# SciML/ExponentialUtilities.jl

Hardware: AMD Instinct MI355X
Metric: expv matvecs/s (Krylov steps/s), n=1e6 5-diagonal sparse fp64, m=30 (higher is better)
Workload: dtype f64; 1 GPU; BASELINE configs[1]: expv(1.0, A, b), n=1000000, offsets (-2..2) diagonals (0.3,1.2,-2.0,0.8,-0.1), nnz=4999994, m=30, tol=1e-7, full Arnoldi (auto), one independent problem per GPU; n=1000000, m=30, nnz=4999994, ortho=auto, entry=expv(t,A,b), outputs=stream-ordered, spinup_calls=535

## Files before the change

### exponentialutilities.jl_amd/_lib.py

```python
import ctypes as C
import os

HERE = os.path.dirname(os.path.abspath(__file__))
LIB_PATH = os.environ.get("EXPV_MI_LIB") or os.path.join(HERE, "libexpv_mi.so")

F64, C64, F32, C32 = 0, 1, 2, 3
HOST, DEVICE = 0, 1
ORTHO_AUTO, ORTHO_MGS, ORTHO_LOWSYNC, ORTHO_PIPELINED = 0, 1, 2, 3
PATH_FLAGS = {"modular": 1, "two_kernel": 2, "pipeline": 4, "wave": 8, "overlapped": 16, "redo_serial": 32,
              "redo_wave_off": 64, "resident": 128, "patch": 256, "pipelined_lanczos": 512}
PATH_FA2_PIPELINED = 1024

STATUS_NAMES = {
    0: "OK", 1: "DimensionMismatch", 2: "ArgumentError", 3: "AssertionError", 4: "SingularException",
    5: "Unsupported", 6: "OutOfMemory", 7: "HIPError", 8: "BoundsError",
}

KERNEL_IDS = {"firststep": 0, "matvec": 1, "dots": 2, "update": 3, "scale": 4, "combine": 5,
              "fused_a": 6, "fused_b": 7, "lincomb": 8, "aug": 9, "batch": 10}


class ArnoldiOpts(C.Structure):
    _fields_ = [("m", C.c_int32), ("iop", C.c_int32), ("init", C.c_int32), ("ishermitian", C.c_int32),
                ("ortho", C.c_int32), ("flags", C.c_int32), ("tol", C.c_double)]


class ExpvStats(C.Structure):
    _fields_ = [("m_used", C.c_int32), ("wasbreakdown", C.c_int32), ("matvecs", C.c_int32),
                ("path_flags", C.c_int32), ("beta", C.c_double)]


ABI_KINDS = {"ArnoldiOpts": 0, "ExpvStats": 1, "TimestepOpts": 2, "TimestepStats": 3, "KiopsOpts": 4}
PRINT_FN = C.CFUNCTYPE(None, C.c_char_p, C.c_void_p)
MATVEC_FN = C.CFUNCTYPE(C.c_int, C.c_void_p, C.c_void_p, C.c_void_p, C.c_void_p)


class TimestepOpts(C.Structure):
    _fields_ = [("tau", C.c_double), ("tol", C.c_double), ("delta", C.c_double), ("gamma", C.c_double),
                ("opnorm", C.c_double), ("has_opnorm", C.c_int32), ("m", C.c_int32), ("iop", C.c_int32),
                ("correct", C.c_int32), ("adaptive", C.c_int32), ("ishermitian", C.c_int32),
                ("verbose", C.c_int32), ("ortho", C.c_int32), ("no_basis_reuse", C.c_int32), ("reserved", C.c_int32),
                ("NA", C.c_int64), ("print", PRINT_FN),
                ("print_user", C.c_void_p)]


class TimestepStats(C.Structure):
    _fields_ = [("num_timesteps", C.c_int32), ("matvecs", C.c_int32), ("m_final", C.c_int32),
                ("arnoldi_calls", C.c_int32), ("arnoldi_reused", C.c_int32), ("stalled_steps", C.c_int32)]


class KiopsOpts(C.Structure):
    _fields_ = [("mmin", C.c_int32), ("mmax", C.c_int32), ("m", C.c_int32), ("iop", C.c_int32),
                ("ishermitian", C.c_int32), ("task1", C.c_int32), ("ortho", C.c_int32),
                ("reserved", C.c_int32), ("tol", C.c_double)]


_vp, _i, _i64, _d = C.c_void_p, C.c_int, C.c_int64, C.c_double
_pi, _pi64, _pd, _pvp = C.POINTER(C.c_int), C.POINTER(C.c_int64), C.POINTER(C.c_double), C.POINTER(C.c_void_p)
PROTOTYPES = {
    "expv_mi_ctx_create": (_i, [_i, _vp, _pvp]),
    "expv_mi_ctx_destroy": (_i, [_vp]),
    "expv_mi_ctx_sync": (_i, [_vp]),
    "expv_mi_ctx_set_async_outputs": (_i, [_vp, _i]),
    "expv_mi_ctx_set_pipeline_overlap": (_i, [_vp, _i]),
    "expv_mi_ctx_counters": (_i, [_vp, _pi64]),
    "expv_mi_ctx_selftest": (_i, [_vp, _pi64]),
    "expv_mi_ctx_set_option": (_i, [_vp, C.c_char_p, _i64]),
    "expv_mi_ctx_get_option": (_i, [_vp, C.c_char_p, _pi64]),
    "expv_mi_last_error": (C.c_char_p, [_vp]),
    "expv_mi_version": (C.c_char_p, []),
    "expv_mi_malloc": (_i, [_vp, C.c_size_t, _pvp]),
    "expv_mi_free": (_i, [_vp, _vp]),
    "expv_mi_memcpy_h2d": (_i, [_vp, _vp, _vp, C.c_size_t]),
    "expv_mi_memcpy_d2h": (_i, [_vp, _vp, _vp, C.c_size_t]),
    "expv_mi_prof_enable": (_i, [_vp, _i]),
    "expv_mi_prof_reset": (_i, [_vp]),
    "expv_mi_prof_get": (_i, [_vp, _i, _pi64, _pd]),
    "expv_mi_prof_name": (C.c_char_p, [_i]),
    "expv_mi_op_create_csc": (_i, [_vp, _i, _i64, _vp, _vp, _vp, _i, _pvp]),
    "expv_mi_op_create_csr": (_i, [_vp, _i, _i64, _vp, _vp, _vp, _i, _i, _pvp]),
    "expv_mi_op_create_csr_loc": (_i, [_vp, _i, _i64, _i64, _vp, _vp, _vp, _i, _i, _i, _pvp]),
    "expv_mi_op_create_csc_loc": (_i, [_vp, _i, _i64, _i64, _vp, _vp, _vp, _i, _i, _i, _pvp]),
    "expv_mi_op_create_coo_loc": (_i, [_vp, _i, _i64, _i64, _vp, _vp, _vp, _i, _i, _i, _pvp]),
    "expv_mi_op_ingest_info": (_i, [_vp, _vp]),
    "expv_mi_op_create_dense": (_i, [_vp, _i, _i64, _vp, _i64, _i, _pvp]),
    "expv_mi_op_create_callback": (_i, [_vp, _i, _i64, MATVEC_FN, _vp, _i, _i64, _pvp]),
    "expv_mi_op_destroy": (_i, [_vp]),
    "expv_mi_op_update_values": (_i, [_vp, _vp, _i]),
    "expv_mi_op_info": (_i, [_vp, _pi64, _pi64, _pi, _pd, _pi]),
    "expv_mi_op_reorder_info": (_i, [_vp, _vp]),
    "expv_mi_op_patch_info": (_i, [_vp, _vp]),
    "expv_mi_plan_cache": (_i, [_i, _i64, _vp]),
    "expv_mi_host_patch_order": (_i, [C.c_int64, _vp, _vp, _i, _vp, _vp, _vp]),
    "expv_mi_host_mesh_patch_order": (_i, [C.c_int64, _vp, _vp, _i, _vp, _vp, _vp]),
    "expv_mi_op_apply": (_i, [_vp, _vp, _i, _vp, _i]),
    "expv_mi_gemv_block": (_i, [_vp, _i, _i64, _i64, _vp, _i64, _vp, _vp, _vp, _i]),
    "expv_mi_expm": (_i, [_vp, _i, _i64, _vp, _i64, _i, _vp]),
    "expv_mi_expm_balanced": (_i, [_vp, _i, _i64, _vp, _i64, _i, _vp]),
    "expv_mi_gebal": (_i, [_vp, _i, _i64, _vp, _i64, _i, _vp, _vp, _vp]),
    "expv_mi_phi": (_i, [_vp, _i, _i64, _i, _vp, _i64, _vp, _i64, _i, _vp]),
    "expv_mi_gemm": (_i, [_vp, _i, _i64, _i64, _i64, _d, _d, _vp, _i64, _vp, _i64, _d, _d, _vp, _i64]),
    "expv_mi_ks_create": (_i, [_vp, _i, _i, _i64, _i, _i, _pvp]),
    "expv_mi_ks_destroy": (_i, [_vp]),
    "expv_mi_ks_resize": (_i, [_vp, _i]),
    "expv_mi_ks_get": (_i, [_vp, _pi, _pi, _pi, _pd, _pi]),
    "expv_mi_ks_set_m": (_i, [_vp, _i]),
    "expv_mi_ks_H": (_i, [_vp, _pvp, _pi, _pi, _pi]),
    "expv_mi_ks_V_download": (_i, [_vp, _i, _i, _vp, _i64]),
    "expv_mi_ks_V_upload": (_i, [_vp, _i, _i, _vp, _i64]),
    "expv_mi_ks_V_devptr": (_i, [_vp, _pvp, _pi64]),
    "expv_mi_arnoldi_opts_default": (None, [C.POINTER(ArnoldiOpts)]),
    "expv_mi_arnoldi": (_i, [_vp, _vp, _vp, _i, C.POINTER(ArnoldiOpts)]),
    "expv_mi_lanczos": (_i, [_vp, _vp, _vp, _i, C.POINTER(ArnoldiOpts)]),
    "expv_mi_arnoldi_aug": (_i, [_vp, _vp, _vp, _i64, _i, _i, _vp, _i, _pd, _d, _d, C.POINTER(ArnoldiOpts)]),
    "expv_mi_expv_ks": (_i, [_vp, _d, _d, _vp, _i, _i]),
    "expv_mi_phiv_ks": (_i, [_vp, _d, _d, _i, _i, _vp, _i64, _i, _i, _pd]),
    "expv_mi_combine": (_i, [_vp, _i, _i, _vp, _i, _i, _d, _vp, _i64, _i, _i]),
    "expv_mi_expv": (_i, [_vp, _vp, _d, _d, _vp, _i, _vp, _i, _i, C.POINTER(ArnoldiOpts), C.POINTER(ExpvStats)]),
    "expv_mi_expv_error_estimate": (_i, [_vp, _vp, _d, _d, _vp, _i, _vp, _i, _d, _d, _i, _i]),
    "expv_mi_timestep_opts_default": (None, [C.POINTER(TimestepOpts)]),
    "expv_mi_timestep_caches_create": (_i, [_vp, _i, _i64, _i, _i, _pvp]),
    "expv_mi_timestep_caches_destroy": (_i, [_vp]),
    "expv_mi_phiv_timestep": (_i, [_vp, _vp, _i, _pd, _vp, _i64, _i, _i, _vp, _i64, _i, C.POINTER(TimestepOpts),
                                   _vp, C.POINTER(TimestepStats)]),
    "expv_mi_kiops_opts_default": (None, [C.POINTER(KiopsOpts)]),
    "expv_mi_kiops": (_i, [_vp, _vp, _pd, _i, _i, _vp, _i64, _i, _i, _vp, _i64, _i, C.POINTER(KiopsOpts), _pi64]),
    "expv_mi_expv_batch": (_i, [_vp, _i, _i64, _i, _vp, _vp, _vp, _i64, _i, _pd, _vp, _i64, _i, _vp, _i64, _i,
                                C.POINTER(ArnoldiOpts), C.POINTER(C.c_int32)]),
    "expv_mi_expv_batch_multi": (_i, [_pvp, _i, _i, _i64, _i, _vp, _vp, _vp, _i64, _pd, _vp, _i64, _vp, _i64, _i,
                                      C.POINTER(ArnoldiOpts), C.POINTER(C.c_int32)]),
    "expv_mi_rccl_available": (_i, []),
    "expv_mi_rccl_unique_id": (_i, [_vp]),
    "expv_mi_comm_create": (_i, [_vp, _vp, _i, _i, _pvp]),
    "expv_mi_gather_rccl": (_i, [_vp, _vp, _vp, _i64, _i]),
    "expv_mi_comm_destroy": (_i, [_vp]),
    "expv_mi_abi_sizeof": (C.c_size_t, [_i]),
    "expv_mi_abi_layout": (C.c_char_p, [_i]),
    "expv_mi_host_pattern_info": (_i, [C.c_int64, _vp, _vp, _i, _vp]),
    "expv_mi_host_rcm": (_i, [C.c_int64, _vp, _vp, _i, _vp, _vp]),
    "expv_mi_host_wrapsum": (_i, [_vp, C.c_uint64, _vp]),
    "expv_mi_host_expm": (_i, [_i, _i, _vp, _i]),
    "expv_mi_host_gebal": (_i, [_i, _i, _vp, _i, _vp, _vp, _vp]),
    "expv_mi_host_symtridiag_expcol": (_i, [_i, _pd, _pd, _d, _d, _pd]),
    "expv_mi_host_symtridiag_exp_last": (_i, [_i, _pd, _pd, _d, _d, _pd]),
    "expv_mi_host_phiv_dense": (_i, [_i, _i, _i, _vp, _i, _vp, _vp]),
}

_lib = None


class ExpvMIError(RuntimeError):
    def __init__(self, code, msg):
        super().__init__(f"{STATUS_NAMES.get(code, code)}: {msg}")
        self.code = code
        self.kind = STATUS_NAMES.get(code, str(code))


def load():
    global _lib
    if _lib is not None:
        return _lib
    if not os.path.exists(LIB_PATH):
        raise ImportError(
            f"{LIB_PATH} is missing: build the HIP extension first "
            "(python -c 'import __graft_entry__ as g; g.build()').  There is no CPU fallback.")
    try:
        import torch
    except ImportError:
        pass
    lib = C.CDLL(LIB_PATH)
    for name, (res, args) in PROTOTYPES.items():
        fn = getattr(lib, name)
        fn.restype = res
        fn.argtypes = args
    _lib = lib
    return lib


def check(code, ctx=None):
    if code != 0:
        msg = load().expv_mi_last_error(ctx)
        raise ExpvMIError(code, msg.decode() if msg else "")
```

### exponentialutilities.jl_amd/api.py

```python
import ctypes as C
import math
import os
import weakref

import numpy as np

from . import _lib as L

__all__ = [
    "Context", "default_context", "MIOperator", "DeviceArray", "KrylovSubspace", "arnoldi", "arnoldi_",
    "lanczos_", "expv", "expv_", "phiv", "phiv_", "expv_timestep", "expv_timestep_", "phiv_timestep",
    "phiv_timestep_", "kiops", "timestep_caches", "expv_batch", "expv_batch_multi", "RcclComm", "rccl_available", "rccl_unique_id", "ExpvMIError", "DimensionMismatch", "host_expm",
    "exponential", "exponential_", "mul_", "phi", "phi_", "balance_", "host_gebal",
    "host_phiv_dense", "host_symtridiag_expcol", "host_symtridiag_exp_last", "host_pattern_info", "host_rcm", "host_patch_order", "clear_operator_cache", "plan_cache",
]

ExpvMIError = L.ExpvMIError


class DimensionMismatch(ValueError):
    """Julia's DimensionMismatch (arnoldi.jl:217-218) -- raised for status 1."""


def _check(code, ctx=None):
    if code == 0:
        return
    try:
        L.check(code, ctx)
    except L.ExpvMIError as e:
        if e.code == 1:
            raise DimensionMismatch(str(e)) from None
        if e.code == 3:
            raise AssertionError(str(e)) from None
        if e.code == 8:
            raise IndexError(str(e)) from None
        raise


class Context:


    def __init__(self, device=None, stream=None, async_outputs=False):
        sptr = None
        if stream is not None:
            handle = getattr(stream, "cuda_stream", stream)
            if not handle:
                raise ValueError("Context(stream=...): the null / legacy stream (handle 0, e.g. torch.cuda.default_stream()) cannot be "
                                 "adopted -- the library would silently work on a stream of its own.  Pass a stream you created "
                                 "(torch.cuda.Stream()), or stream=None for a private stream of the library's.")
            sptr = C.c_void_p(int(handle))
        lib = L.load()
        if device is None:
            device = int(os.environ.get("LOCAL_RANK", "0"))
        h = C.c_void_p()
        _check(lib.expv_mi_ctx_create(int(device), sptr, C.byref(h)))
        self._h = h
        self.device = int(device)
        self._stream_keepalive = stream
        self._finalizer = weakref.finalize(self, lib.expv_mi_ctx_destroy, h)
        self._async_outputs = bool(async_outputs)
        if async_outputs:
            _check(lib.expv_mi_ctx_set_async_outputs(h, 1))

    def sync(self):
        _check(L.load().expv_mi_ctx_sync(self._h), self._h)

    def set_async_outputs(self, on=True):
        _check(L.load().expv_mi_ctx_set_async_outputs(self._h, int(bool(on))), self._h)
        self._async_outputs = bool(on)

    def set_option(self, name, value):
        _check(L.load().expv_mi_ctx_set_option(self._h, name.encode(), int(value)), self._h)

    def get_option(self, name):
        v = C.c_int64(0)
        _check(L.load().expv_mi_ctx_get_option(self._h, name.encode(), C.byref(v)), self._h)
        return int(v.value)

    def selftest(self):
        out = (C.c_int64 * 8)()
        _check(L.load().expv_mi_ctx_selftest(self._h, out), self._h)
        return tuple(int(x) for x in out)

    def counters(self):
        out = (C.c_int64 * 8)()
        _check(L.load().expv_mi_ctx_counters(self._h, out), self._h)
        keys = ("krylov_steps", "factorisations", "pipeline", "overlapped", "redo_serial", "redo_wave_off", "op_applies", "h_by_copy")
        return dict(zip(keys, (int(v) for v in out)))

    def set_pipeline_overlap(self, on=True):
        _check(L.load().expv_mi_ctx_set_pipeline_overlap(self._h, int(bool(on))), self._h)

    def prof_enable(self, on=True):
        L.load().expv_mi_prof_enable(self._h, int(bool(on)))

    def prof_reset(self):
        _check(L.load().expv_mi_prof_reset(self._h), self._h)

    def prof_get(self):
        out = {}
        for name, kid in L.KERNEL_IDS.items():
            n, ms = C.c_int64(0), C.c_double(0.0)
            _check(L.load().expv_mi_prof_get(self._h, kid, C.byref(n), C.byref(ms)), self._h)
            if n.value:
                out[name] = {"launches": int(n.value), "total_ms": float(ms.value)}
        return out


_default_ctx = None


def default_context():
    global _default_ctx
    if _default_ctx is None:
        _default_ctx = Context()
    return _default_ctx


class DeviceArray:

    def __init__(self, shape, dtype, ctx=None):
        self.ctx = ctx or default_context()
        self.shape = tuple(int(s) for s in (shape if isinstance(shape, (tuple, list)) else (shape,)))
        self.dtype = np.dtype(dtype)
        nbytes = int(np.prod(self.shape)) * self.dtype.itemsize
        p = C.c_void_p()
        _check(L.load().expv_mi_malloc(self.ctx._h, nbytes, C.byref(p)), self.ctx._h)
        self.ptr = p.value
        self.nbytes = nbytes
        self._finalizer = weakref.finalize(self, L.load().expv_mi_free, self.ctx._h, p)

    @classmethod
    def from_host(cls, a, ctx=None):
        a = np.asfortranarray(a)
        d = cls(a.shape, a.dtype, ctx)
        _check(L.load().expv_mi_memcpy_h2d(d.ctx._h, d.ptr, a.ctypes.data, a.nbytes), d.ctx._h)
        return d

    def to_host(self):
        out = np.empty(self.shape, dtype=self.dtype, order="F")
        _check(L.load().expv_mi_memcpy_d2h(self.ctx._h, out.ctypes.data, self.ptr, self.nbytes), self.ctx._h)
# ... 1357 lines not shown
    if x.dim() != 2 or _dense_np_dtype(x) != dt:
        raise TypeError(f"mul_: {what} must be a 2-D tensor of dtype {dt}")
    return None, None, tuple(x.shape), x


def mul_(Cm, A, B, alpha=1, beta=0, ctx=None):
    dt = _dense_np_dtype(Cm)
    args = [_dense_dev_arg(x, dt, w) for x, w in ((Cm, "C"), (A, "A"), (B, "B"))]
    (m, n), (ma, k), (kb, nb) = (tuple(int(v) for v in a[2]) for a in args)
    if ma != m or kb != k or nb != n:
        raise DimensionMismatch(f"mul!: C is {m}x{n}, A is {ma}x{k}, B is {kb}x{nb}")
    alpha, beta = complex(alpha), complex(beta)
    if dt.kind != "c" and (alpha.imag != 0 or beta.imag != 0):
        raise TypeError("InexactError: complex scalar with a real element type")
    ptrs, keep = [], []
    for i, (ptr, ld, shape, x) in enumerate(args):
        if ptr is None:
            if not (x.stride(0) == 1 and (shape[1] <= 1 or x.stride(1) >= max(shape[0], 1))) and min(shape) > 0:
                if i == 0:
                    raise TypeError("output matrix must be column-major (e.g. torch.empty(n, m).t())")
                x = x.t().contiguous().t()
            keep.append(x)
            ptr, ld = x.data_ptr(), (x.stride(1) if shape[1] > 1 else max(shape[0], 1))
        ptrs.append((ptr, max(int(ld), 1)))
    tens = [x for x in keep if _is_torch(x)]
    if tens:
        _torch_ready(*tens)
    c = ctx or (Cm.ctx if isinstance(Cm, DeviceArray) else default_context())
    _check(L.load().expv_mi_gemm(c._h, _code(dt), m, n, k, alpha.real, alpha.imag, ptrs[1][0], ptrs[1][1], ptrs[2][0], ptrs[2][1],
                                 beta.real, beta.imag, ptrs[0][0], ptrs[0][1]), c._h)
    if not getattr(c, "_async_outputs", False):
        c.sync()
    return Cm


def _host_dtype(*dts):
    dt = np.result_type(*[np.dtype(d) for d in dts])
    if dt.kind not in "fc" or dt.itemsize < 4:
        dt = np.result_type(dt, np.float64)
    if dt.itemsize > 16 or (dt.kind == "f" and dt.itemsize > 8):
        dt = np.dtype(np.complex128 if dt.kind == "c" else np.float64)
    if dt == np.dtype(np.float16):
        dt = np.dtype(np.float32)
    return dt


def host_expm(A):
    A = np.array(A, dtype=_host_dtype(np.asarray(A).dtype), order="F", copy=True)
    n = A.shape[0]
    _check(L.load().expv_mi_host_expm(_HOST_CODES[A.dtype], n, A.ctypes.data, max(n, 1)))
    return A


def host_gebal(A):
    A = np.array(A, dtype=_host_dtype(np.asarray(A).dtype), order="F", copy=True)
    if A.ndim != 2 or A.shape[0] != A.shape[1]:
        raise DimensionMismatch(f"host_gebal: matrix is not square: dimensions are {A.shape}")
    n = A.shape[0]
    ilo, ihi = C.c_int64(1), C.c_int64(0)
    scale = np.ones(n, dtype=np.float64)
    _check(L.load().expv_mi_host_gebal(_HOST_CODES[A.dtype], n, A.ctypes.data, max(n, 1), C.byref(ilo), C.byref(ihi), scale.ctypes.data))
    return A, int(ilo.value), int(ihi.value), scale


def host_pattern_info(A, dtype=np.float64):
    import scipy.sparse as sp
    A = sp.csr_matrix(A)
    n = A.shape[0]
    rp = np.ascontiguousarray(A.indptr, dtype=np.int32)
    ci = np.ascontiguousarray(A.indices, dtype=np.int32)
    out = np.zeros(8, dtype=np.int64)
    _check(L.load().expv_mi_host_pattern_info(n, rp.ctypes.data, ci.ctypes.data, _code(np.dtype(dtype)), out.ctypes.data))
    info = {"sell": bool(out[0]), "bandwidth": int(out[1]), "pipeline_dia_diagonals": int(out[2]),
            "general_dia_diagonals": int(out[3]), "general_dia_max_offset": int(out[4]), "sell_wave_reach": int(out[5]),
            "rows_sorted_unique": bool(out[6]), "sell_cut": int(out[7])}
    if not info["sell"]:
        info["path"] = "modular (empty operator)"
    elif info["sell_cut"] > 0:
        info["path"] = "two-kernel step, SELL slots up to the cut + overflow pass (irregular rows)"
    elif info["pipeline_dia_diagonals"] or (np.dtype(dtype) in (np.dtype(np.float64), np.dtype(np.float32)) and info["bandwidth"] <= 8):
        info["path"] = "pipeline, halo form"
    elif np.dtype(dtype) in (np.dtype(np.float64), np.dtype(np.float32)) and (info["general_dia_diagonals"] or info["sell_wave_reach"] >= 0):
        info["path"] = ("pipeline, wave form (when the reach is small against the resident grid), else two-kernel step; a 2-D grid "
                        "stencil: pipeline, patch form under context option patch (host_patch_order)")
    else:
        info["path"] = "two-kernel step"
    return info


def host_rcm(A, dtype=np.float64):
    import scipy.sparse as sp
    A = sp.csr_matrix(A)
    n = A.shape[0]
    rp = np.ascontiguousarray(A.indptr, dtype=np.int32)
    ci = np.ascontiguousarray(A.indices, dtype=np.int32)
    perm = np.zeros(n, dtype=np.int32)
    out = np.zeros(4, dtype=np.int64)
    _check(L.load().expv_mi_host_rcm(n, rp.ctypes.data, ci.ctypes.data, _code(np.dtype(dtype)), perm.ctypes.data, out.ctypes.data))
    names = {3: "single-pass step, halo form", 2: "single-pass step, wave form", 1: "two-kernel step", 0: "two-kernel step + overflow pass"}
    return perm, {"bandwidth_before": int(out[0]), "bandwidth_after": int(out[1]), "form_before": names[int(out[2]) & 255],
                  "form_after": names[int(out[3])], "would_reorder": bool(int(out[2]) & 256)}


def host_patch_order(A, dtype=np.float64, mesh=False):
    import scipy.sparse as sp
    A = sp.csr_matrix(A)
# ... 46 lines not shown
```

### exponentialutilities.jl_amd/csrc/capi.hip

```cpp
#include <algorithm>
#include <chrono>
#include <climits>
#include <cmath>
#include <mutex>
#include <thread>
#include <cstddef>
#include <type_traits>
#include <cstring>
#include <dlfcn.h>
#include <functional>
#include <unordered_map>

#include "engine.h"
#include "reorder.h"

using namespace expv_mi;
using dense::cd;
using dense::Mat;

namespace {
thread_local std::string g_last_error;

template <class F>
int guarded(Ctx *ctx, F &&f) {
// ... 1110 lines not shown
    if (!op.csc_pos.empty()) {
      op.csc_pos_dev.alloc(sizeof(int32_t) * op.csc_pos.size());
      HIPCHECK(hipMemcpyAsync(op.csc_pos_dev.p, op.csc_pos.data(), sizeof(int32_t) * op.csc_pos.size(), hipMemcpyHostToDevice, s));
      dev::op_scatter_values<T>(s, op.val.as<T>(), reinterpret_cast<const T *>(vals), op.csc_pos_dev.as<int32_t>(), op.nnz);
    } else {
      HIPCHECK(hipMemcpyAsync(op.val.p, vals, sizeof(V) * ci.size(), hipMemcpyDeviceToDevice, s));
    }
  }
  lap("CSR arrays + values in place");
  const PatternPlan P = pc.get(n, rp, ci, (int)sizeof(V));
  build_csr_layouts<V>(op, n, rp, ci, P, lap);
  unsigned long long out[32];
  op_fill_forms<T>(op, true, op.rows_sorted_unique, out);
  lap("device fill of the forms");
  double opn;
  std::memcpy(&opn, &out[0], sizeof(double));
  op.opnorm_inf = opn;
  if (op.rows_sorted_unique) {
    op.ishermitian = out[1] ? 0 : 1;
  } else {
    std::vector<V> va(ci.size());
    if (!va.empty()) HIPCHECK(hipMemcpy(va.data(), op.val.p, sizeof(V) * va.size(), hipMemcpyDeviceToHost));
    double dummy;
    csr_props<V>(n, rp, ci, va, &op.ishermitian, &dummy);
    op.ingest[2] = (int64_t)(sizeof(V) * va.size());
  }
  upload_tile_ranges<V>(op, n, rp, ci, P);
}

void check_device_dtype(int dt, const char *who) {
  if (dt != EXPV_MI_F64 && dt != EXPV_MI_C64 && dt != EXPV_MI_F32 && dt != EXPV_MI_C32)
    fail(EXPV_MI_ARGUMENT_ERROR, std::string(who) + ": unknown dtype");
}
void check_64bit_dtype(int dt, const char *who) {
  check_device_dtype(dt, who);
  if (dtype_is_32bit(dt)) fail(EXPV_MI_UNSUPPORTED, std::string(who) + ": Float64 / ComplexF64 only");
}

const char *kKernelNames[EXPV_MI_K_COUNT] = {"firststep", "matvec", "dots",    "update", "scale", "combine",
                                             "fused_a",   "fused_b", "lincomb", "aug",    "batch"};
}

namespace {
template <class S>
void host_expm_T(int n, void *A, int lda) {
  Mat<S> M(n, n);
  for (int j = 0; j < n; ++j)
    for (int i = 0; i < n; ++i) M(i, j) = reinterpret_cast<S *>(A)[(size_t)j * lda + i];
  dense::expm_higham2005base(M);
  for (int j = 0; j < n; ++j)
    for (int i = 0; i < n; ++i) reinterpret_cast<S *>(A)[(size_t)j * lda + i] = M(i, j);
}
template <class S>
void host_gebal_T(int n, void *A, int lda, int64_t *ilo, int64_t *ihi, double *scale) {
  Mat<S> M(n, n);
  for (int j = 0; j < n; ++j)
    for (int i = 0; i < n; ++i) M(i, j) = reinterpret_cast<S *>(A)[(size_t)j * lda + i];
  const dense::Balance<S> B = dense::gebal(M);
  for (int j = 0; j < n; ++j)
    for (int i = 0; i < n; ++i) reinterpret_cast<S *>(A)[(size_t)j * lda + i] = M(i, j);
  if (ilo) *ilo = B.ilo;
  if (ihi) *ihi = B.ihi;
  if (scale)
    for (int i = 0; i < n; ++i) scale[i] = (double)B.scale[(size_t)i];
}
template <class S>
void host_phiv_dense_T(int m, int k, const void *A, int lda, const void *v, void *w) {
  Mat<S> M(m, m);
  std::vector<S> vv(m);
  for (int j = 0; j < m; ++j)
    for (int i = 0; i < m; ++i) M(i, j) = reinterpret_cast<const S *>(A)[(size_t)j * lda + i];
  for (int i = 0; i < m; ++i) vv[i] = reinterpret_cast<const S *>(v)[i];
  Mat<S> R = dense::phiv_dense(M, vv, k);
  std::copy(R.a.begin(), R.a.end(), reinterpret_cast<S *>(w));
}
}

template <class T, class V>
static void op_update_values_T(Op &op, const void *vals, int loc) {
  Ctx *c = op.ctx;
  hipStream_t s = c->stream;
  const int64_t nnz = op.nnz;
  const T *src = reinterpret_cast<const T *>(vals);
  if (loc == EXPV_MI_HOST) {
    if (op.upd_stage.bytes < sizeof(T) * (size_t)nnz) op.upd_stage.alloc(sizeof(T) * (size_t)nnz + 16);
    HIPCHECK(hipMemcpyAsync(op.upd_stage.p, vals, sizeof(T) * (size_t)nnz, hipMemcpyHostToDevice, s));
    src = op.upd_stage.as<T>();
  }
  if (!op.csc_pos.empty()) {
    if (!op.csc_pos_dev.p) {
      op.csc_pos_dev.alloc(sizeof(int32_t) * op.csc_pos.size());
      HIPCHECK(hipMemcpyAsync(op.csc_pos_dev.p, op.csc_pos.data(), sizeof(int32_t) * op.csc_pos.size(), hipMemcpyHostToDevice, s));
    }
    dev::op_scatter_values<T>(s, op.val.as<T>(), src, op.csc_pos_dev.as<int32_t>(), nnz);
  } else {
    HIPCHECK(hipMemcpyAsync(op.val.p, src, sizeof(T) * (size_t)nnz, hipMemcpyDeviceToDevice, s));
  }
  unsigned long long out[32];
  op_fill_forms<T>(op, false, op.rows_sorted_unique, out);
  double opn;
  std::memcpy(&opn, &out[0], sizeof(double));
  op.opnorm_inf = opn;
  if (op.rows_sorted_unique) {
    op.ishermitian = out[1] ? 0 : 1;
  } else {
    std::vector<int32_t> rp((size_t)op.n + 1), ci((size_t)nnz);
// ... 62 lines not shown
  (void)hipSetDevice(ctx->device);
  for (auto &p : ctx->prof)
    for (auto &ev : p.ev) { (void)hipEventDestroy(ev.first); (void)hipEventDestroy(ev.second); }
  ht_report();
  ctx->orphan_children();
  delete reinterpret_cast<expv_mi_ks_s *>(ctx->ws_ks);
  if (ctx->ws_kiops && ctx->ws_kiops_free) ctx->ws_kiops_free(ctx->ws_kiops);
  delete reinterpret_cast<expv_mi_ks_s *>(ctx->ks_spare);
  if (ctx->ws_ts && ctx->ws_ts_free) ctx->ws_ts_free(ctx->ws_ts);
  if (ctx->ws_batch_pat && ctx->ws_batch_pat_free) ctx->ws_batch_pat_free(ctx->ws_batch_pat);
  if (ctx->ws_batch && ctx->ws_batch_free) ctx->ws_batch_free(ctx->ws_batch);
  if (ctx->ws_dense && ctx->ws_dense_free) ctx->ws_dense_free(ctx->ws_dense);
  for (auto &sp : ctx->stage_spares) (void)hipFree(sp.p);
  ctx->stage_spares.clear();
  if (ctx->stream2) (void)hipStreamDestroy(ctx->stream2);
  if (ctx->ev_fork) (void)hipEventDestroy(ctx->ev_fork);
  if (ctx->ev_join) (void)hipEventDestroy(ctx->ev_join);
  if (ctx->owns_stream && ctx->stream) (void)hipStreamDestroy(ctx->stream);
  delete ctx;
  return EXPV_MI_OK;
}
int expv_mi_ctx_set_async_outputs(expv_mi_ctx_t ctx, int on) {
  if (!ctx) return EXPV_MI_ARGUMENT_ERROR;
  ctx->async_out = (on != 0);
  return EXPV_MI_OK;
}
int expv_mi_ctx_set_pipeline_overlap(expv_mi_ctx_t ctx, int on) {
  if (!ctx) return EXPV_MI_ARGUMENT_ERROR;
  ctx->pipe_overlap = (on != 0);
  return EXPV_MI_OK;
}
int expv_mi_ctx_set_option(expv_mi_ctx_t ctx, const char *name, int64_t value) {
  if (!ctx) return EXPV_MI_ARGUMENT_ERROR;
  return guarded(ctx, [&] {
    int *slot = ctx->opt.find(name);
    if (!slot) fail(EXPV_MI_ARGUMENT_ERROR, std::string("unknown option: ") + (name ? name : "(null)"));
    if (value < 0 || value > INT_MAX) fail(EXPV_MI_ARGUMENT_ERROR, "option value out of range");
    *slot = (int)value;
    if (slot == &ctx->opt.batch_rounds && *slot < 1) *slot = 1;
  });
}
int expv_mi_ctx_get_option(expv_mi_ctx_t ctx, const char *name, int64_t *value) {
  if (!ctx || !value) return EXPV_MI_ARGUMENT_ERROR;
  return guarded(ctx, [&] {
    int *slot = ctx->opt.find(name);
    if (!slot) fail(EXPV_MI_ARGUMENT_ERROR, std::string("unknown option: ") + (name ? name : "(null)"));
    *value = *slot;
  });
}
int expv_mi_ctx_counters(expv_mi_ctx_t ctx, int64_t out[8]) {
  if (!ctx || !out) return EXPV_MI_ARGUMENT_ERROR;
  out[0] = ctx->cnt_steps; out[1] = ctx->cnt_fact; out[2] = ctx->cnt_pipe; out[3] = ctx->cnt_live;
  out[4] = ctx->cnt_serial_redo; out[5] = ctx->cnt_wave_redo; out[6] = ctx->cnt_opapply; out[7] = ctx->cnt_copy;
  return EXPV_MI_OK;
}
int expv_mi_ctx_selftest(expv_mi_ctx_t ctx, int64_t out[8]) {
  if (!out) return EXPV_MI_ARGUMENT_ERROR;
  return guarded(ctx, [&] {
    ctx->use();
    const size_t nin = (size_t)32 * dev::BLOCK;
    std::vector<double> h(nin);
    uint64_t x = 0x9e3779b97f4a7c15ull;
    for (size_t i = 0; i < nin; ++i) {
      x ^= x << 13; x ^= x >> 7; x ^= x << 17;
      const double u = (double)(x >> 11) * (1.0 / 9007199254740992.0) - 0.5;
      h[i] = std::ldexp(u, (int)((x >> 3) % 40) - 20);
    }
    double *din = nullptr;
    unsigned long long *dout = nullptr;
    HIPCHECK(hipMalloc((void **)&din, nin * sizeof(double)));
    HIPCHECK(hipMalloc((void **)&dout, 8 * sizeof(unsigned long long)));
    unsigned long long res[8] = {0, 0, 0, 0, 0, 0, 0, 0};
    hipError_t e = hipMemcpyAsync(din, h.data(), nin * sizeof(double), hipMemcpyHostToDevice, ctx->stream);
    if (e == hipSuccess) e = hipMemsetAsync(dout, 0, sizeof(res), ctx->stream);
    if (e == hipSuccess) { dev::selftest_lanes(ctx->stream, din, dout); e = hipGetLastError(); }
    if (e == hipSuccess) e = hipMemcpyAsync(res, dout, sizeof(res), hipMemcpyDeviceToHost, ctx->stream);
    if (e == hipSuccess) e = hipStreamSynchronize(ctx->stream);
    (void)hipFree(din);
    (void)hipFree(dout);
    HIPCHECK(e);
    for (int i = 0; i < 8; ++i) out[i] = (int64_t)res[i];
  });
}
int expv_mi_ctx_sync(expv_mi_ctx_t ctx) {
  return guarded(ctx, [&] { ctx->use(); HIPCHECK(hipStreamSynchronize(ctx->stream)); });
}
const char *expv_mi_last_error(expv_mi_ctx_t ctx) { return ctx ? ctx->last_error.c_str() : g_last_error.c_str(); }

int expv_mi_malloc(expv_mi_ctx_t ctx, size_t bytes, void **dptr) {
  return guarded(ctx, [&] { ctx->use(); HIPCHECK(hipMalloc(dptr, bytes ? bytes : 1)); });
}
int expv_mi_free(expv_mi_ctx_t, void *dptr) {
  return guarded(nullptr, [&] { if (dptr) HIPCHECK(hipFree(dptr)); });
}
int expv_mi_memcpy_h2d(expv_mi_ctx_t ctx, void *dst, const void *src, size_t bytes) {
  return guarded(ctx, [&] {
    ctx->use();
    HIPCHECK(hipMemcpyAsync(dst, src, bytes, hipMemcpyHostToDevice, ctx->stream));
    HIPCHECK(hipStreamSynchronize(ctx->stream));
  });
}
int expv_mi_memcpy_d2h(expv_mi_ctx_t ctx, void *dst, const void *src, size_t bytes) {
  return guarded(ctx, [&] {
    ctx->use();
    HIPCHECK(hipMemcpyAsync(dst, src, bytes, hipMemcpyDeviceToHost, ctx->stream));
    HIPCHECK(hipStreamSynchronize(ctx->stream));
// ... 1081 lines not shown
int expv_mi_host_rcm(int64_t n, const int32_t *rowptr, const int32_t *colind, int dtype, int32_t *perm, int64_t out[4]) {
  return guarded(nullptr, [&] {
    if (n < 0 || !rowptr || (n > 0 && rowptr[n] > 0 && !colind)) fail(EXPV_MI_ARGUMENT_ERROR, "host_rcm: bad arguments");
    check_device_dtype(dtype, "host_rcm");
    check_host_pattern(n, rowptr, colind, "host_rcm");
    const int64_t nnz = n > 0 ? (int64_t)rowptr[n] : 0;
    const std::vector<int32_t> pv = reorder::rcm(n, rowptr, colind);
    if (perm) std::copy(pv.begin(), pv.end(), perm);
    if (out) {
      std::vector<int32_t> rp2, ci2, src;
      reorder::permute_csr(n, rowptr, colind, pv, rp2, ci2, src);
      const PatternPlan P0 = analyze_pattern(n, rowptr, colind, nnz, (int)dtype_size(dtype));
      const PatternPlan P1 = analyze_pattern(n, rp2.data(), ci2.data(), nnz, (int)dtype_size(dtype));
      out[0] = P0.bandwidth;
      out[1] = P1.bandwidth;
      const PatClass c0 = pattern_class_ex(P0, n, dtype), c1 = pattern_class_ex(P1, n, dtype);
      const bool candidate = c0.cls == 1 || (c0.cls == 2 && !c0.dia && c0.reach > 4096);
      const bool better = c1.cls > c0.cls || (c1.cls == c0.cls && c1.cls == 2 && 4 * c1.reach <= c0.reach);
      out[2] = (n > 0 ? c0.cls : 1) | ((n > 0 && candidate && better) ? 256 : 0);
      out[3] = n > 0 ? c1.cls : 1;
    }
  });
}
static int host_patch_order_impl(int64_t n, const int32_t *rowptr, const int32_t *colind, int dtype, int32_t *perm, int32_t *ring_count, int64_t out[8], bool mesh) {
  return guarded(nullptr, [&] {
    if (n < 0 || !rowptr || (n > 0 && rowptr[n] > 0 && !colind) || !out) fail(EXPV_MI_ARGUMENT_ERROR, "host_patch_order: bad arguments");
    check_device_dtype(dtype, "host_patch_order");
    check_host_pattern(n, rowptr, colind, "host_patch_order");
    for (int q = 0; q < 8; ++q) out[q] = 0;
    PatchPlan pl;
    const int64_t nnz = n > 0 ? (int64_t)rowptr[n] : 0;
    if (mesh ? !plan_mesh_patch(n, rowptr, colind, nnz, (int)dtype_size(dtype), 0, pl) : !plan_patch(n, rowptr, colind, nnz, (int)dtype_size(dtype), pl)) return;
    if (perm) std::copy(pl.perm.begin(), pl.perm.end(), perm);
    if (ring_count) std::copy(pl.cnt.begin(), pl.cnt.end(), ring_count);
    out[0] = 1; out[1] = pl.k; out[2] = pl.nt; out[3] = pl.maxring; out[4] = pl.ring_sum; out[5] = pl.over128;
    out[6] = (int64_t)pl.lcol.size(); out[7] = pl.RP;
  });
}
int expv_mi_host_patch_order(int64_t n, const int32_t *rowptr, const int32_t *colind, int dtype, int32_t *perm, int32_t *ring_count, int64_t out[8]) {
  return host_patch_order_impl(n, rowptr, colind, dtype, perm, ring_count, out, false);
}
int expv_mi_host_mesh_patch_order(int64_t n, const int32_t *rowptr, const int32_t *colind, int dtype, int32_t *perm, int32_t *ring_count, int64_t out[8]) {
  return host_patch_order_impl(n, rowptr, colind, dtype, perm, ring_count, out, true);
}
int expv_mi_host_expm(int dtype, int n, void *A, int lda) {
  return guarded(nullptr, [&] {
    if (n < 0 || lda < n || (n > 0 && !A)) fail(EXPV_MI_ARGUMENT_ERROR, "host_expm: bad n / lda / A");
    switch (dtype) {
      case EXPV_MI_F64: host_expm_T<double>(n, A, lda); break;
      case EXPV_MI_C64: host_expm_T<cd>(n, A, lda); break;
      case EXPV_MI_F32: host_expm_T<float>(n, A, lda); break;
      case EXPV_MI_C32: host_expm_T<dense::cf>(n, A, lda); break;
      default: fail(EXPV_MI_ARGUMENT_ERROR, "host_expm: unknown dtype");
    }
  });
}
int expv_mi_host_gebal(int dtype, int n, void *A, int lda, int64_t *ilo, int64_t *ihi, double *scale) {
  return guarded(nullptr, [&] {
    if (n < 0 || lda < n || (n > 0 && !A)) fail(EXPV_MI_ARGUMENT_ERROR, "host_gebal: bad n / lda / A");
    switch (dtype) {
      case EXPV_MI_F64: host_gebal_T<double>(n, A, lda, ilo, ihi, scale); break;
      case EXPV_MI_C64: host_gebal_T<cd>(n, A, lda, ilo, ihi, scale); break;
      case EXPV_MI_F32: host_gebal_T<float>(n, A, lda, ilo, ihi, scale); break;
      case EXPV_MI_C32: host_gebal_T<dense::cf>(n, A, lda, ilo, ihi, scale); break;
      default: fail(EXPV_MI_ARGUMENT_ERROR, "host_gebal: unknown dtype");
    }
  });
}
int expv_mi_host_symtridiag_expcol(int n, const double *d, const double *e, double t_re, double t_im, double *out_c64) {
  return guarded(nullptr, [&] {
    std::vector<double> dv(d, d + n), ev(e, e + (n > 1 ? n - 1 : 0));
    std::vector<cd> r = dense::symtridiag_expcol<cd>(dv, ev, cd(t_re, t_im));
    for (int i = 0; i < n; ++i) { out_c64[2 * i] = r[i].real(); out_c64[2 * i + 1] = r[i].imag(); }
  });
}
int expv_mi_host_symtridiag_exp_last(int n, const double *d, const double *e, double t_re, double t_im, double *out_c64) {
  return guarded(nullptr, [&] {
    if (n < 1) fail(EXPV_MI_ARGUMENT_ERROR, "symtridiag_exp_last: n >= 1 required");
    std::vector<double> dv(d, d + n), ev(e, e + (n > 1 ? n - 1 : 0));
    const cd r = dense::symtridiag_exp_last<cd>(dv, ev, cd(t_re, t_im));
    out_c64[0] = r.real();
    out_c64[1] = r.imag();
  });
}
int expv_mi_host_phiv_dense(int dtype, int m, int k, const void *A, int lda, const void *v, void *w) {
  return guarded(nullptr, [&] {
    switch (dtype) {
      case EXPV_MI_F64: host_phiv_dense_T<double>(m, k, A, lda, v, w); break;
      case EXPV_MI_C64: host_phiv_dense_T<cd>(m, k, A, lda, v, w); break;
      case EXPV_MI_F32: host_phiv_dense_T<float>(m, k, A, lda, v, w); break;
      case EXPV_MI_C32: host_phiv_dense_T<dense::cf>(m, k, A, lda, v, w); break;
      default: fail(EXPV_MI_ARGUMENT_ERROR, "host_phiv_dense: unknown dtype");
    }
  });
}

int expv_mi_expv_batch(expv_mi_ctx_t ctx, int dtype, int64_t n, int nprob, const int32_t *rowptr, const int32_t *colind,
                       const void *vals, int64_t nnz_per_prob, int mat_loc, const double *t, const void *b, int64_t ldb,
                       int b_loc, void *w, int64_t ldw, int w_loc, const expv_mi_arnoldi_opts *opts, int32_t *m_used) {
  return guarded(ctx, [&] {
    check_device_dtype(dtype, "expv_batch");
    expv_mi_arnoldi_opts o;
    if (opts) o = *opts; else expv_mi_arnoldi_opts_default(&o);
    expv_batch_run(ctx, dtype, n, nprob, rowptr, colind, vals, nnz_per_prob, mat_loc, t, b, ldb, b_loc, w, ldw, w_loc, o,
                   m_used);
  });
// ... 193 lines not shown
```

### exponentialutilities.jl_amd/csrc/engine.h

```cpp
#pragma once
#include <hip/hip_runtime.h>

#include <complex>
#include <cstdint>
#include <cstdio>
#include <cstring>
#include <memory>
#include <mutex>
#include <string>
#include <vector>

#include "../../include/expv_mi.h"
#include "device_types.h"
#include "host_dense.h"
#include "kernels.h"

namespace expv_mi {

struct Err {
  int code;
  std::string msg;
};
[[noreturn]] inline void fail(int code, const std::string &m) { throw Err{code, m}; }

// ... 56 lines not shown
  int ee_blocked = 1;
  int reorder = 1;
  int patch = 1;
  int matfree_fused = 0;
  int fa2_pipelined = 1;
  int kiops_skip_redo = 1;
  int resident = 0;
  static Options from_env();
  int *find(const char *name);
};

struct Ctx {
  int device = 0;
  Options opt;
  hipStream_t stream = nullptr;
  bool owns_stream = false;
  std::string last_error;
  bool prof_on = false;
  bool async_out = false;
  bool pipe_overlap = true;
  ProfSlot prof[EXPV_MI_K_COUNT];
  void *ws_ks = nullptr;
  void *ws_kiops = nullptr;
  void (*ws_kiops_free)(void *) = nullptr;
  void *ks_spare = nullptr;
  std::vector<Ctx **> children;
  std::mutex children_mu;
  void adopt(Ctx **slot) {
    std::lock_guard<std::mutex> g(children_mu);
    children.push_back(slot);
  }
  void release(Ctx **slot) {
    std::lock_guard<std::mutex> g(children_mu);
    for (size_t i = 0; i < children.size(); ++i)
      if (children[i] == slot) { children[i] = children.back(); children.pop_back(); return; }
  }
  void orphan_children() {
    std::lock_guard<std::mutex> g(children_mu);
    for (Ctx **slot : children) *slot = nullptr;
    children.clear();
  }
  void *ws_ts = nullptr;
  void (*ws_ts_free)(void *) = nullptr;
  void *ws_batch_pat = nullptr;
  void (*ws_batch_pat_free)(void *) = nullptr;
  void *ws_batch = nullptr;
  size_t ws_batch_bytes = 0;
  void (*ws_batch_free)(void *) = nullptr;
  void *ws_dense = nullptr;
  void (*ws_dense_free)(void *) = nullptr;
  int dense_force_singular = 0;
  int dense_tile = 0;
  int64_t cnt_steps = 0, cnt_fact = 0, cnt_live = 0, cnt_serial_redo = 0, cnt_wave_redo = 0, cnt_opapply = 0, cnt_pipe = 0, cnt_copy = 0;
  int last_path = 0;
  hipStream_t stream2 = nullptr;
  hipEvent_t ev_fork = nullptr, ev_join = nullptr;
  void ensure_aux() {
    if (stream2) return;
    HIPCHECK(hipStreamCreateWithFlags(&stream2, hipStreamNonBlocking));
    HIPCHECK(hipEventCreateWithFlags(&ev_fork, hipEventDisableTiming));
    HIPCHECK(hipEventCreateWithFlags(&ev_join, hipEventDisableTiming));
  }
  void use() const { HIPCHECK(hipSetDevice(device)); }
  struct Spare { void *p; size_t bytes; };
  std::vector<Spare> stage_spares;
  void *stage_take(size_t need, size_t *got) {
    *got = 0;
    if (need == 0) return nullptr;
    for (size_t i = 0; i < stage_spares.size(); ++i)
      if (stage_spares[i].bytes >= need && stage_spares[i].bytes <= 4 * need + ((size_t)1 << 20)) {
        void *q = stage_spares[i].p;
        *got = stage_spares[i].bytes;
        stage_spares[i] = stage_spares.back();
        stage_spares.pop_back();
        return q;
      }
    void *q = nullptr;
    HIPCHECK(hipMalloc(&q, need));
    *got = need;
    return q;
  }
  void stage_give(void *p, size_t bytes) {
    if (stage_spares.size() < 4 && bytes <= ((size_t)1 << 30)) { stage_spares.push_back(Spare{p, bytes}); return; }
    (void)hipFree(p);
  }
};
}
struct expv_mi_ctx_s : expv_mi::Ctx {};
namespace expv_mi {

struct DevBuf {
  void *p = nullptr;
  size_t bytes = 0;
  Ctx *home = nullptr;
  DevBuf() {}
  explicit DevBuf(size_t b) { alloc(b); }
  DevBuf(const DevBuf &) = delete;
  DevBuf &operator=(const DevBuf &) = delete;
  DevBuf(DevBuf &&o) noexcept : p(o.p), bytes(o.bytes), home(o.home) { o.p = nullptr; o.bytes = 0; o.home = nullptr; }
  DevBuf &operator=(DevBuf &&o) noexcept {
    if (this != &o) { release(); p = o.p; bytes = o.bytes; home = o.home; o.p = nullptr; o.bytes = 0; o.home = nullptr; }
    return *this;
  }
  void alloc(size_t b) {
    release();
    bytes = b;
// ... 106 lines not shown
  std::shared_ptr<RowPerm> perm;
};
}
struct expv_mi_op_s : expv_mi::Op {};
namespace expv_mi {

struct Ks {
  Ctx *ctx = nullptr;
  int device = 0;
  int dtypeT = EXPV_MI_F64, dtypeU = EXPV_MI_F64;
  int64_t n = 0;
  int maxiter = 30, augmented = 0;
  int m = 30;
  double beta = 0.0;
  bool wasbreakdown = false;
  int64_t ldv = 0;
  DevBuf V;
  std::vector<char> H;
  int ldh = 0, hcols = 0;
  DevBuf Hdev;
  int ldhd = 0;
  DevBuf gram;
  int ldg = 0;
  int gram_rows = 0;
  DevBuf hcoef, part, gpart, state;
  DevBuf plbuf;
  StepState state_host;
  void *pin = nullptr;
  size_t pin_bytes = 0;
  ~Ks() {
    if (!ctx) b_stored.home = nullptr;
    if (pin) (void)hipHostFree(pin);
    if (mbox) (void)hipHostFree(mbox);
  }
  DevBuf hcoef2, colscale;
  DevBuf flags;
  DevBuf tflags;
  bool lanczos_continue = false;
  uint32_t pipe_seq = 0;
  bool pipe_resident_used = false;
  bool pipe_serial = false, pipe_live_used = false;
  int pipe_serial_calls = 0;
  bool wave_off = false;
  int wave_off_calls = 0;
  void *mbox = nullptr, *mbox_dev = nullptr;
  size_t mbox_bytes = 0;
  bool mbox_armed = false;
  bool defer_tail_req = false;
  struct TailPending { bool pending = false, lanczos = false; int m = 0; uint32_t seq = 0; void *stream = nullptr; } tail;
  bool pipe_closed = false;
  std::vector<double> colscale_host;
  bool scale_pending = false;
  bool skip_tail = false;
  int scale_cols = 0;
  DevBuf ubuf, ybuf;
  DevBuf extbuf;
  std::shared_ptr<RowPerm> vperm;
  bool b_natural = false;
  DevBuf b_stored;
  int64_t rows() const { return n + augmented; }
};
void ks_finish_tail(Ks &ks);
struct TailDrain {
  Ks &k;
  ~TailDrain() { try { ks_finish_tail(k); } catch (...) {} }
};
void ks_recycle(Ks &ks);
}
struct expv_mi_ks_s : expv_mi::Ks {};
namespace expv_mi {

struct TsCache {
  Ctx *ctx = nullptr;
  int device = 0;
  int dtype = EXPV_MI_F64;
  int64_t n = 0;
  int maxiter = 0, p = 0;
  DevBuf u, W, P;
  expv_mi_ks_s *ks = nullptr;
};
}
struct expv_mi_tscache_s : expv_mi::TsCache {};
namespace expv_mi {

inline dense::cd getH(const Ks &ks, int i, int j) {
  const size_t e = (size_t)j * ks.ldh + i;
  switch (ks.dtypeU) {
    case EXPV_MI_C64: { const double *p = reinterpret_cast<const double *>(ks.H.data()) + 2 * e; return dense::cd(p[0], p[1]); }
    case EXPV_MI_F32: return dense::cd((double)reinterpret_cast<const float *>(ks.H.data())[e], 0.0);
    case EXPV_MI_C32: { const float *p = reinterpret_cast<const float *>(ks.H.data()) + 2 * e; return dense::cd((double)p[0], (double)p[1]); }
    default: return dense::cd(reinterpret_cast<const double *>(ks.H.data())[e], 0.0);
  }
}
inline void setH(Ks &ks, int i, int j, dense::cd v) {
  const size_t e = (size_t)j * ks.ldh + i;
  switch (ks.dtypeU) {
    case EXPV_MI_C64: { double *p = reinterpret_cast<double *>(ks.H.data()) + 2 * e; p[0] = v.real(); p[1] = v.imag(); } break;
    case EXPV_MI_F32: reinterpret_cast<float *>(ks.H.data())[e] = (float)v.real(); break;
    case EXPV_MI_C32: { float *p = reinterpret_cast<float *>(ks.H.data()) + 2 * e; p[0] = (float)v.real(); p[1] = (float)v.imag(); } break;
    default: reinterpret_cast<double *>(ks.H.data())[e] = v.real(); break;
  }
}
inline void setH_realpart(Ks &ks, int i, int j, double v) {
  const size_t e = (size_t)j * ks.ldh + i;
  switch (ks.dtypeU) {
    case EXPV_MI_C64: reinterpret_cast<double *>(ks.H.data())[2 * e] = v; break;
// ... 68 lines not shown
```

### exponentialutilities.jl_amd/csrc/engine_core.hip

```cpp
#include <cstdlib>

#include <atomic>
#include <chrono>
#include <cstdio>

#include <type_traits>

#include "engine.h"

namespace expv_mi {

using dense::cd;
using dense::Mat;

static inline int64_t round_up(int64_t x, int64_t a) { return (x + a - 1) / a * a; }

const void *stage_in(Ctx *ctx, const void *p, int loc, size_t bytes, DevBuf &tmp) {
  if (loc == EXPV_MI_DEVICE || bytes == 0) return p;
  tmp.take_from(ctx, bytes);
  HIPCHECK(hipMemcpyAsync(tmp.p, p, bytes, hipMemcpyHostToDevice, ctx->stream));
  HIPCHECK(hipStreamSynchronize(ctx->stream));
  return tmp.p;
}

// ... 92 lines not shown
  ks.Hdev.alloc((size_t)ks.ldhd * (ks.maxiter + 1) * esz + 8);
  HIPCHECK(hipMemsetAsync(ks.Hdev.p, 0, ks.Hdev.bytes, ks.ctx->stream));
  ks.ldg = ks.maxiter + 1;
  ks.gram.alloc((size_t)ks.ldg * ks.ldg * esz);
  HIPCHECK(hipMemsetAsync(ks.gram.p, 0, ks.gram.bytes, ks.ctx->stream));
  ks.hcoef.alloc((size_t)(ks.maxiter + 2) * esz);
  if (!ks.part.p) ks.part.alloc((size_t)(dev::MAX_RED_VALUES + 8) * dev::MAX_GRID * sizeof(double));
  if (!ks.gpart.p) ks.gpart.alloc((size_t)(dev::MAX_RED_VALUES + 8) * dev::MAX_GROUPS * sizeof(double));
  const size_t state_bytes = sizeof(StepState) + sizeof(uint32_t) * (size_t)dev::PIPE_ARRIVE_STEP * (size_t)(std::max(ks.maxiter, dev::PIPE_CH) + 3);
  if (ks.state.bytes < state_bytes) {
    ks.state.alloc(state_bytes);
    HIPCHECK(hipMemsetAsync(ks.state.p, 0, state_bytes, ks.ctx->stream));
  }
}

void ks_alloc(Ks &ks, Ctx *ctx, int dtT, int dtU, int64_t n, int maxiter, int augmented) {
  if (n < 0 || maxiter < 1 || augmented < 0) fail(EXPV_MI_ARGUMENT_ERROR, "KrylovSubspace: bad n/maxiter/augmented");
  for (int dt : {dtT, dtU})
    if (dt != EXPV_MI_F64 && dt != EXPV_MI_C64 && dt != EXPV_MI_F32 && dt != EXPV_MI_C32) fail(EXPV_MI_ARGUMENT_ERROR, "KrylovSubspace: unknown dtype");
  if (!dtype_is_complex(dtT) && dtype_is_complex(dtU)) fail(EXPV_MI_ARGUMENT_ERROR, "KrylovSubspace: U complex with T real");
  if (dtype_is_32bit(dtT) != dtype_is_32bit(dtU)) fail(EXPV_MI_ARGUMENT_ERROR, "KrylovSubspace: T and U must have the same precision (U = T or real(T))");
  ctx->use();
  ks.ctx = ctx;
  ks.dtypeT = dtT;
  ks.dtypeU = dtU;
  ks.n = n;
  ks.maxiter = ks.m = maxiter;
  ks.augmented = augmented;
  ks.beta = 0.0;
  ks.wasbreakdown = false;
  ks.ldv = round_up(ks.rows() > 0 ? ks.rows() : 1, dtype_row_pad(dtT));
  const size_t esz = dtype_size(dtT);
  ks.V.alloc((size_t)ks.ldv * (maxiter + 1) * esz);
  HIPCHECK(hipMemsetAsync(ks.V.p, 0, ks.V.bytes, ctx->stream));
  ks.ldh = maxiter + 1;
  ks.hcols = maxiter + (augmented != 0 ? 1 : 0);
  ks.H.assign((size_t)ks.ldh * ks.hcols * dtype_size(dtU), 0);
  ks.gram_rows = 0;
  ks_alloc_aux(ks);
  HIPCHECK(hipStreamSynchronize(ctx->stream));
}

void ks_recycle(Ks &ks) {
  ks.ctx->use();
  if (ks.tail.pending) ks_finish_tail(ks);
  ks.m = ks.maxiter;
  ks.beta = 0.0;
  ks.wasbreakdown = false;
  std::fill(ks.H.begin(), ks.H.end(), 0);
  ks.gram_rows = 0;
  ks.scale_pending = false;
  ks.scale_cols = 0;
  ks.skip_tail = false;
  ks.defer_tail_req = false;
  ks.pipe_closed = false;
  ks.mbox_armed = false;
  ks.vperm.reset();
  hipStream_t s = ks.ctx->stream;
  HIPCHECK(hipMemsetAsync(ks.Hdev.p, 0, ks.Hdev.bytes, s));
  HIPCHECK(hipMemsetAsync(ks.gram.p, 0, ks.gram.bytes, s));
  HIPCHECK(hipMemsetAsync(ks.state.p, 0, ks.state.bytes, s));
}

void ks_resize(Ks &ks, int maxiter) {
  ks.ctx->use();
  ks_materialize(ks);
  const bool isaug = ks.augmented != 0;
  const size_t esz = dtype_size(ks.dtypeT), usz = dtype_size(ks.dtypeU);
  DevBuf Vn((size_t)ks.ldv * (maxiter + 1) * esz);
  HIPCHECK(hipMemsetAsync(Vn.p, 0, Vn.bytes, ks.ctx->stream));
  const int ldh_n = maxiter + 1, hcols_n = maxiter + (isaug ? 1 : 0);
  std::vector<char> Hn((size_t)ldh_n * hcols_n * usz, 0);
  DevBuf gram_old = std::move(ks.gram);
  const int ldg_old = ks.ldg, mi_old = ks.maxiter;
  if (isaug) {
    const int ccopy = std::min(ks.maxiter + 1, maxiter + 1);
    HIPCHECK(hipMemcpyAsync(Vn.p, ks.V.p, (size_t)ks.ldv * ccopy * esz, hipMemcpyDeviceToDevice, ks.ctx->stream));
    const int rc = std::min(ks.ldh, ldh_n), cc = std::min(ks.hcols, hcols_n);
    for (int j = 0; j < cc; ++j)
      std::memcpy(&Hn[(size_t)j * ldh_n * usz], &ks.H[(size_t)j * ks.ldh * usz], (size_t)rc * usz);
  }
  HIPCHECK(hipStreamSynchronize(ks.ctx->stream));
  ks.V = std::move(Vn);
  ks.H.swap(Hn);
  ks.ldh = ldh_n;
  ks.hcols = hcols_n;
  ks.m = ks.maxiter = maxiter;
  ks_alloc_aux(ks);
  if (isaug) {
    const int q = std::min(mi_old + 1, maxiter + 1);
    HIPCHECK(hipMemcpy2DAsync(ks.gram.p, (size_t)ks.ldg * esz, gram_old.p, (size_t)ldg_old * esz, (size_t)q * esz, q,
                              hipMemcpyDeviceToDevice, ks.ctx->stream));
  } else {
    ks.gram_rows = 0;
  }
  HIPCHECK(hipStreamSynchronize(ks.ctx->stream));
}

void ks_materialize(Ks &ks) {
  if (!ks.scale_pending) return;
  ks.ctx->use();
  if (ks.scale_cols > 0) {
    dispatch_dtype(ks.dtypeT, [&](auto tag) {
      using T = typename decltype(tag)::type;
      dev::scale_columns<T>(ks.ctx->stream, ks.V.as<T>(), ks.ldv, ks.rows(), ks.colscale.as<double>(), ks.scale_cols);
    });
  }
  HIPCHECK(hipStreamSynchronize(ks.ctx->stream));
  ks.scale_pending = false;
  ks.scale_cols = 0;
}

template <class T>
static dev::OvfView<T> ovf_view(const Op &op) {
  return dev::OvfView<T>{op.ovf_seg.as<int32_t>(), op.ovf_nseg, op.ovf_piece.as<int32_t>(), op.ovf_multi.as<int32_t>(), op.ovf_nmulti,
                         op.ovf_part.as<T>(), op.ovf_col.as<int32_t>(), op.ovf_val.as<T>(), op.ovf_y.as<T>(),
                         op.cbf_row16.as<uint16_t>(), op.cbf_P.as<T>(), op.cbf_pstride, op.cbf ? op.cbf_ncb : 0, op.n};
}
// ... 147 lines not shown
  if (!g_ht_on) return;
  const auto now = std::chrono::steady_clock::now();
  if (id > 0) { g_ht_sum[id] += std::chrono::duration<double, std::micro>(now - g_ht_last).count(); g_ht_cnt[id]++; }
  g_ht_last = now;
}
void ht_report() {
  if (!g_ht_on) return;
  static const char *names[16] = {"", "front (reset, fork)", "step launches + join", "H/state read-back + sync", "scales read-back + sync",
                                  "host exp(tH)", "combine launch", "H copy + structure checks", "combine: coefficient prep", "", "", "", "", "", "", ""};
  for (int i = 1; i < 16; ++i)
    if (g_ht_cnt[i]) std::fprintf(stderr, "[host timing] %-28s %8.2f us avg over %ld\n", names[i], g_ht_sum[i] / g_ht_cnt[i], g_ht_cnt[i]);
}
thread_local CallTrace *t_call_trace = nullptr;
bool CallTrace::enabled() {
  static const bool e = std::getenv("EXPV_MI_CALL_TRACE") != nullptr;
  return e;
}
void CallTrace::mark(const char *what) {
  if (!on) return;
  ev.emplace_back(what, std::chrono::duration<double, std::micro>(std::chrono::steady_clock::now().time_since_epoch()).count());
}
void CallTrace::dump(const char *title) {
  if (!on || ev.empty()) return;
  std::fprintf(stderr, "[call trace] %s\n", title);
  for (size_t i = 0; i < ev.size(); ++i)
    std::fprintf(stderr, "[call trace] %9.1f us  +%7.1f  %s\n", ev[i].second - ev[0].second, i ? ev[i].second - ev[i - 1].second : 0.0, ev[i].first);
  ev.clear();
}
template <class T>
static int arnoldi_T(Ks &ks, Op &op, const T *b, const expv_mi_arnoldi_opts &o, const ArnoldiAug *aug, bool lanczos);
template <class T> constexpr bool kPipeType = true;

template <class T>
struct ArnoldiCall {
  Ks &ks;
  Op &op;
  const T *b;
  const expv_mi_arnoldi_opts &o;
  const ArnoldiAug *aug;
  const bool lanczos;
  Ctx *c;
  hipStream_t s;
  const bool isaug, real_coeff, no_dia_env;
  const int p;
  const double tol;
  int init;
  const bool fresh;
  int m = 0, iop = 0, jstart = 1, hview_rows = 0, hview_cols = 0;
  int64_t rows = 0, wave_reach = 0;
  T *V = nullptr, *Hd = nullptr, *hcoef = nullptr;
  StepState *st = nullptr;
  double *part = nullptr, *gpart = nullptr;
  bool h_zeroed = false;
  bool fa2_pl_used = false;
  bool cont_reset_done = false;
  bool tail_deferred = false;
  bool use_fused = false, single_red = false, use_pipe = false, use_wave = false, use_ring = false, mbox_generic = false;
  const int32_t *b_map = nullptr;
  bool b_nat = false;

  ArnoldiCall(Ks &ks_, Op &op_, const T *b_, const expv_mi_arnoldi_opts &o_, const ArnoldiAug *aug_, bool lanczos_)
      : ks(ks_), op(op_), b(b_), o(o_), aug(aug_), lanczos(lanczos_), c(ks_.ctx), s(ks_.ctx->stream), isaug(aug_ != nullptr),
        real_coeff(dtype_is_complex(ks_.dtypeT) && !dtype_is_complex(ks_.dtypeU)), no_dia_env(!ks_.ctx->opt.dia),
        p(aug_ ? aug_->p : 0), tol(o_.tol), init(o_.init), fresh(o_.init == 0) {}

  int run() {
    c->use();
    m = o.m > 0 ? o.m : (int)std::min<int64_t>(ks.maxiter, op.n);
    ks.wasbreakdown = false;
    if (init == 0) { ks.scale_pending = false; ks.scale_cols = 0; }
    if (m > ks.maxiter) ks_resize(ks, m);
    else ks.m = m;
    if (op.n != ks.n || p != ks.augmented)
      fail(EXPV_MI_DIMENSION_MISMATCH, "length(b') == size(A,1) == size(A,2) == size(V,1)-p doesn't hold");
    if (op.dtype != ks.dtypeT) fail(EXPV_MI_ARGUMENT_ERROR, "operator dtype must equal the subspace dtype T");
    rows = ks.rows();
    V = ks.V.as<T>();
    st = ks.state.as<StepState>();
    hview_rows = m + 1;
    hview_cols = m + (isaug ? 1 : 0);

    choose_step_form();
    if (ks.b_natural) {
      ks.b_natural = false;
      b_nat = true;
      if (fresh && ks.vperm) {
        if (use_pipe && !isaug && !c->opt.resident && g_perm_fused) b_map = ks.vperm->p.as<int32_t>();
        else {
          int64_t ld = ks.n;
          b = reinterpret_cast<const T *>(permute_in(c, *ks.vperm, b, EXPV_MI_DEVICE, 1, ks.n, sizeof(T), ks.b_stored, &ld));
          b_nat = false;
        }
      }
    }
    if constexpr (std::is_same<T, double>::value) {
      if (lanczos_pipelined_applies()) {
        const int r = run_lanczos_pipelined();
        if (r >= 0) return r;
      }
    }
    if (fresh) first_step();
    if (ks.beta == 0.0) return 0;
    iop = o.iop;
    if (iop == 0) iop = m;
    jstart = (lanczos && !ks.lanczos_continue) ? 1 : init;
    if (jstart > m) return 0;
    ct_mark("  arnoldi!: form chosen, first step set up");
    reset_device_state();
    ct_mark("  arnoldi!: device state reset enqueued");
    if (use_pipe) {
      if constexpr (kPipeType<T>) steps_single_pass();
      else fail(EXPV_MI_HIP_ERROR, "single-pass step chosen for a 32-bit element type");
    }
    else if (use_fused && single_red) steps_two_kernel();
    else if (use_fused) steps_two_kernel_two_reductions();
    else steps_modular();
    ct_mark("  arnoldi!: all step launches enqueued");
    return read_back();
  }

  bool lanczos_pipelined_applies() const {
    return lanczos && o.ortho == EXPV_MI_ORTHO_PIPELINED && fresh && !isaug && op.kind == OP_CSR && op.ndiag > 0 && !no_dia_env &&
           op.bandwidth >= 1 && op.bandwidth <= dev::PIPE_WMAX && ks.dtypeT == EXPV_MI_F64 && !b_nat && b_map == nullptr && m >= 1 && m <= dev::PL_MAX_M &&
           ks.n >= 2 * dev::PIPE_WMAX * 3 && !c->prof_on;
  }
  int run_lanczos_pipelined() {
    if constexpr (!std::is_same<T, double>::value) return -1;
    else {
    const int cap = dev::lanczos_pl_capacity();
    if (cap <= 0) return -1;
    const size_t part_b = sizeof(double) * 4 * 12 * (size_t)dev::MAX_GRID, cnt_b = sizeof(uint32_t) * (size_t)(dev::PL_MAX_M + 8),
                 flag_b = sizeof(uint32_t) * 2 * (size_t)dev::MAX_GRID, out_n = 8 + 2 * (size_t)(dev::PL_MAX_M + 3) + 8, out_b = sizeof(double) * out_n;
    if (ks.plbuf.bytes < part_b + cnt_b + flag_b + out_b) ks.plbuf.alloc(part_b + cnt_b + flag_b + out_b);
    char *base = ks.plbuf.as<char>();
    dev::LanczosPlArgs a{};
    a.dia_val = op.dia_val.as<double>(); a.dia_ld = op.dia_ld; a.ndiag = op.ndiag;
    for (int d = 0; d < op.ndiag; ++d) a.dia_off[d] = op.dia_off[d];
    a.w = (int)op.bandwidth;
    a.n_dia = op.dia_ld;
    a.V = ks.V.as<double>(); a.ldv = ks.ldv; a.n = ks.n;
    a.u0 = reinterpret_cast<const double *>(b);
    a.part = reinterpret_cast<double *>(base);
    a.count = reinterpret_cast<uint32_t *>(base + part_b);
    a.flags = reinterpret_cast<uint32_t *>(base + part_b + cnt_b);
    a.out = reinterpret_cast<double *>(base + part_b + cnt_b + flag_b);
    a.m = m; a.want_tail = ks.skip_tail ? 0 : 1; a.tol = tol; a.spin_limit = c->opt.spin_limit;
    HIPCHECK(hipMemsetAsync(base + part_b, 0, cnt_b + flag_b + out_b, s));
    for (int j = 0; j < hview_cols; ++j)
      std::memset(&ks.H[(size_t)j * ks.ldh * dtype_size(ks.dtypeU)], 0, (size_t)hview_rows * dtype_size(ks.dtypeU));
    if (!dev::lanczos_pl(s, a)) return -1;
    const size_t need = out_b;
    if (ks.pin_bytes < need) {
      if (ks.pin) (void)hipHostFree(ks.pin);
      ks.pin = nullptr;
      ks.pin_bytes = std::max(need, sizeof(T) * (size_t)ks.ldhd * (ks.maxiter + 1) + sizeof(StepState));
      HIPCHECK(hipHostMalloc(&ks.pin, ks.pin_bytes, hipHostMallocDefault));
    }
    double *out = reinterpret_cast<double *>(ks.pin);
    HIPCHECK(hipMemcpyAsync(out, a.out, out_b, hipMemcpyDeviceToHost, s));
    HIPCHECK(hipStreamSynchronize(s));
    ks.scale_pending = false;
    ks.scale_cols = 0;
    ks.gram_rows = 0;
    ks.tail.pending = false;
    if (out[2] != 0.0) { ++c->cnt_serial_redo; return -1; }
    ks.beta = std::sqrt(out[0]);
    if (ks.beta == 0.0) return 0;
    const int md = (int)out[1];
    const int jlast = md > 0 ? std::min(md, m) : m;
    const double *al = out + 8, *be = out + 8 + dev::PL_MAX_M + 3;
// ... 12 lines not shown
    }
  }

  void choose_step_form() {
    const bool no_fused = !c->opt.fused;
    single_red = !c->opt.fused_two_reductions;
    const bool stored = (op.kind == OP_CSR) && op.sell_ok && (single_red || op.sell_cut == 0);
    const bool matfree = (op.kind == OP_CALLBACK) && single_red && c->opt.matfree_fused;
    use_fused = !no_fused && (stored || matfree) && (!isaug || (single_red && p <= dev::FUSED_AUG_MAX)) &&
                o.ortho != EXPV_MI_ORTHO_MGS && (lanczos || std::min(o.iop == 0 ? m : o.iop, m) <= dev::LOWSYNC_MAX);
    const bool no_pipe = !c->opt.pipeline;
    {
      const int iopw = lanczos ? 2 : (o.iop == 0 ? m : std::min(o.iop, m));
      const int wstep = std::min(m - 1, iopw);
      const bool have_dia = op.ndiag > 0 && !no_dia_env;
      use_pipe = kPipeType<T> && use_fused && single_red && !no_pipe && op.sell_cut == 0 && op.bandwidth >= 0 && op.bandwidth <= dev::PIPE_WMAX &&
                 wstep <= dev::pipe_max_window<T>() && m + 2 <= dev::PIPE_MAX_STEPS &&
                 (have_dia || ((std::is_same<T, double>::value || std::is_same<T, float>::value) && !isaug)) &&
                 (!isaug || !dtype_is_32bit(ks.dtypeT)) &&
                 (!isaug || (p <= dev::PIPE_AUG_MAX && std::min(m, iopw) <= 7));
      {
        if ((!use_pipe || !have_dia) && op.ring_pad > 0 && c->opt.patch && use_fused && single_red && !no_pipe && op.sell_cut == 0 &&
            wstep <= dev::pipe_max_window<T>() && m + 2 <= dev::PIPE_MAX_STEPS &&
            (!isaug || (!dtype_is_32bit(ks.dtypeT) && p <= dev::PIPE_AUG_MAX && std::min(m, iopw) <= 7))) {
          use_pipe = true;
          use_ring = true;
        }
      }
  }
  if constexpr (std::is_same<T, double>::value || std::is_same<T, float>::value) {
    const bool no_wave = !c->opt.wave;
    const int64_t trw = (int64_t)(16 / sizeof(T)) * dev::BLOCK;
    const int64_t ntiles_w = (ks.n + trw - 1) / trw;
    if (ks.wave_off && ++ks.wave_off_calls > 64) { ks.wave_off = false; ks.wave_off_calls = 0; }
    const bool wave_dia = op.gndiag > 0 && !no_dia_env;
    const bool wave_sell = !wave_dia && op.tile_reach >= 0;
    const int64_t reach_rows = wave_dia ? op.gdia_maxoff : op.tile_reach;
    if (!use_pipe && use_fused && single_red && !isaug && !no_pipe && !no_wave && !ks.wave_off && (wave_dia || wave_sell) &&
        m <= dev::PIPE_CH && !real_coeff && fresh && (ntiles_w <= 400 || (reach_rows / trw + 2) * 4 <= 400)) {
      use_pipe = true;
      use_wave = true;
      wave_reach = reach_rows;
    }
  }
  if (!fresh) {
    if (!single_red) use_fused = use_pipe = false;
    const int wcont = lanczos ? 2 : std::min(o.iop == 0 ? m : o.iop, m);
    if (!lanczos && wcont >= 3 && ks.gram_rows < init - 1) use_fused = use_pipe = false;
    if (!use_fused) use_pipe = false;
    if (!use_pipe) ks_materialize(ks);
  }
  }

  void first_step() {
    for (int j = 0; j < hview_cols; ++j)
      std::memset(&ks.H[(size_t)j * ks.ldh * dtype_size(ks.dtypeU)], 0, (size_t)hview_rows * dtype_size(ks.dtypeU));
    dev::zero_two(s, st, ks.state.bytes, ks.Hdev.as<T>() + (size_t)(jstart - 1) * ks.ldhd, sizeof(T) * (size_t)ks.ldhd * (m - jstart + 1));
    h_zeroed = true;
    double extra = 0.0;
    const T *src = b;
    if (isaug) {
      for (int k = 1; k <= p; ++k) {
        if (k == p) aug->w_aug_host[k - 1] = aug->mu;
        else {
          const int i = p - k;
          double f = 1.0;
          for (int q = 2; q <= i; ++q) f *= q;
          aug->w_aug_host[k - 1] = std::pow(aug->t, i) / f * aug->mu;
        }
        extra += aug->w_aug_host[k - 1] * aug->w_aug_host[k - 1];
      }
      src = reinterpret_cast<const T *>(aug->w);
  }
  if (use_pipe) {
  } else if (use_fused && single_red) {
    HIPCHECK(hipMemcpyAsync(V, src, sizeof(T) * (size_t)ks.n, hipMemcpyDeviceToDevice, s));
    if (isaug) {
      std::vector<T> tail(p);
      for (int k = 0; k < p; ++k) tail[k] = ST<T>::from_real(aug->w_aug_host[k]);
      HIPCHECK(hipMemcpyAsync(V + ks.n, tail.data(), sizeof(T) * p, hipMemcpyHostToDevice, s));
      HIPCHECK(hipStreamSynchronize(s));
    }
  } else {
    ProfScope ps(c, EXPV_MI_K_FIRSTSTEP);
    dev::sumsq<T>(s, src, ks.n, ks.part.as<double>(), ks.gpart.as<double>(), st);
  }
  ks.gram_rows = 0;
  if (use_fused) {
    ks.beta = 1.0;
  } else {
    StepState h;
    read_state<T>(ks, &h);
    ks.beta = std::sqrt(h.sumsq + extra);
  }
  if (ks.beta != 0.0 && use_fused) {
    ks.gram_rows = 1;
  } else if (ks.beta != 0.0) {
    ProfScope ps(c, EXPV_MI_K_FIRSTSTEP);
    if (isaug) {
      dev::scale_copy<T>(s, V, src, ks.n, ks.beta, 1);
      std::vector<T> tail(p);
      for (int k = 0; k < p; ++k) tail[k] = ST<T>::from_real(aug->w_aug_host[k] / ks.beta);
      HIPCHECK(hipMemcpyAsync(V + ks.n, tail.data(), sizeof(T) * p, hipMemcpyHostToDevice, s));
      HIPCHECK(hipStreamSynchronize(s));
    } else {
      dev::scale_copy<T>(s, V, src, ks.n, 1.0 / ks.beta, 0);
    }
    ks.gram_rows = 1;
  }
  init = 1;
// ... 426 lines not shown
  if (((use_pipe && ks.pipe_live_used) || mbox_generic) && ks.mbox_armed) {
    const MailboxView mvh = mailbox_view(ks, ks.mbox);
    const double *mh = mvh.H;
    const size_t hwords = mailbox_hwords(ks), swords = (size_t)ks.maxiter + 2;
    const bool defer = ks.defer_tail_req && use_pipe && ks.pipe_live_used && ks.pipe_closed && !ks.pipe_resident_used && !mbox_generic;
    const volatile unsigned long long *done = defer ? mvh.done + 1 : mvh.done;
    tail_deferred = false;
    for (long it = 1;; ++it) {
      if (*done == (unsigned long long)ks.pipe_seq) { from_mbox = true; break; }
      __builtin_ia32_pause();
      if ((it & 0xfff) == 0) {
        const hipError_t q = hipStreamQuery(s);
        if (q == hipSuccess) {
          from_mbox = (*done == (unsigned long long)ks.pipe_seq);
          break;
        }
        if (q != hipErrorNotReady) HIPCHECK(q);
      }
    }
    if (from_mbox) {
      std::atomic_thread_fence(std::memory_order_acquire);
      Hh = reinterpret_cast<const T *>(mh);
      std::memset(&h, 0, sizeof(h));
      h.beta0sq = mh[hwords + swords];
      h.breakdown = (int32_t)mh[hwords + swords + 1];
      h.m_done = (int32_t)mh[hwords + swords + 2];
      tail_deferred = defer && h.breakdown == 0;
    }
  }
  if (!from_mbox) {
    HIPCHECK(hipMemcpyAsync(ks.pin, Hd, hbytes, hipMemcpyDeviceToHost, s));
    HIPCHECK(hipMemcpyAsync(&h, st, sizeof(StepState), hipMemcpyDeviceToHost, s));
    HIPCHECK(hipStreamSynchronize(s));
  }
  ht_mark(3);
  if (h.breakdown == 99) {
    if (use_wave && !ks.wave_off) {
      ks.wave_off = true;
      ks.wave_off_calls = 0;
      ++c->cnt_wave_redo;
      ks.b_natural = b_nat;
      const int r = arnoldi_T<T>(ks, op, b, o, aug, lanczos);
      c->last_path |= EXPV_MI_PATH_REDO_WAVE_OFF;
      return r;
    }
    if (!ks.pipe_live_used || ks.pipe_serial) fail(EXPV_MI_HIP_ERROR, "pipelined factorisation: bounded wait expired");
    ks.pipe_serial = true;
    ++c->cnt_serial_redo;
    ks.b_natural = b_nat;
    const int r = arnoldi_T<T>(ks, op, b, o, aug, lanczos);
    c->last_path |= EXPV_MI_PATH_REDO_SERIAL;
    return r;
  }
  if (use_fused && fresh) {
    ks.beta = std::sqrt(h.beta0sq);
    if (ks.beta == 0.0) { ks.gram_rows = 0; return 0; }
  }
  if (use_pipe) {
    const int ncol = ((h.breakdown == 1) ? h.m_done + 1 : ((ks.skip_tail || tail_deferred) ? m : m + 1));
    ks.colscale_host.assign(ks.maxiter + 2, 1.0);
    if (from_mbox) {
      const double *ms = mailbox_view(ks, ks.mbox).scales;
      for (int q = 0; q < ncol; ++q) ks.colscale_host[q] = ms[q];
    } else {
      HIPCHECK(hipMemcpyAsync(ks.colscale_host.data(), ks.colscale.p, sizeof(double) * (size_t)ncol, hipMemcpyDeviceToHost, s));
      HIPCHECK(hipStreamSynchronize(s));
    }
    ht_mark(4);
    ks.scale_pending = true;
    ks.scale_cols = ncol;
  }
  const int jlast = (h.breakdown == 1) ? h.m_done : m;
  auto toc = [](const T &v) -> cd {
    if constexpr (ST<T>::is_complex) return cd(v.re, v.im);
    else return cd(v, 0.0);
  };
  if (lanczos) {
    for (int j = 1; j <= jlast; ++j) {
      setH(ks, j - 1, j - 1, toc(Hh[(size_t)(j - 1) * ks.ldhd + (j - 1)]));
      if (!(tail_deferred && j == m)) setH_realpart(ks, j, j - 1, toc(Hh[(size_t)(j - 1) * ks.ldhd + j]).real());
    }
    const int nsub = std::min(hview_rows - 1, hview_cols);
    for (int i = 1; i < nsub; ++i)
      if (i < hview_cols) setH(ks, i - 1, i, cd(getH(ks, i, i - 1).real(), 0.0));
  } else {
    const int iopw = iop;
    for (int j = jstart; j <= jlast; ++j) {
      const int i0 = std::max(1, j - iopw + 1);
      for (int i = i0; i <= j; ++i) setH(ks, i - 1, j - 1, toc(Hh[(size_t)(j - 1) * ks.ldhd + (i - 1)]));
      if (!(tail_deferred && j == m)) setH(ks, j, j - 1, toc(Hh[(size_t)(j - 1) * ks.ldhd + j]));
    }
  }
  ks.tail.pending = tail_deferred;
  if (tail_deferred) { ks.tail.lanczos = lanczos; ks.tail.m = m; ks.tail.seq = ks.pipe_seq; ks.tail.stream = (void *)s; }
  if (h.breakdown == 1) {
    ks.m = h.m_done;
    ks.wasbreakdown = true;
  }
  c->cnt_steps += jlast - jstart + 1;
  ++c->cnt_fact;
  c->last_path = use_pipe ? (EXPV_MI_PATH_PIPELINE | (use_wave ? EXPV_MI_PATH_WAVE : 0) | (use_ring ? EXPV_MI_PATH_PATCH : 0) | (ks.pipe_live_used ? EXPV_MI_PATH_OVERLAPPED : 0) | (ks.pipe_resident_used ? EXPV_MI_PATH_RESIDENT : 0))
                          : (use_fused ? (EXPV_MI_PATH_TWO_KERNEL | (fa2_pl_used ? EXPV_MI_PATH_FA2_PIPELINED : 0)) : EXPV_MI_PATH_MODULAR);
  if (!from_mbox) ++c->cnt_copy;
  if (use_pipe) { ++c->cnt_pipe; if (ks.pipe_live_used) ++c->cnt_live; }
  return jlast - jstart + 1;
  }
// ... 28 lines not shown
  const size_t hwords = mailbox_hwords(ks), swords = (size_t)ks.maxiter + 2;
  const double *mh = mv.H;
  const size_t e = (size_t)(m - 1) * ks.ldhd + m;
  cd v;
  switch (ks.dtypeT) {
    case EXPV_MI_C64: v = cd(mh[2 * e], mh[2 * e + 1]); break;
    case EXPV_MI_F32: v = cd((double)reinterpret_cast<const float *>(mh)[e], 0.0); break;
    case EXPV_MI_C32: v = cd((double)reinterpret_cast<const float *>(mh)[2 * e], (double)reinterpret_cast<const float *>(mh)[2 * e + 1]); break;
    default: v = cd(mh[e], 0.0); break;
  }
  if (ks.tail.lanczos) setH_realpart(ks, m, m - 1, v.real()); else setH(ks, m, m - 1, v);
  if ((int)ks.colscale_host.size() > m) ks.colscale_host[m] = mv.scales[m];
  ks.scale_cols = m + 1;
  if ((int32_t)mh[hwords + swords + 1] == 1) ks.wasbreakdown = true;
}

int arnoldi_run(Ks &ks, Op &op, const void *b_dev, const expv_mi_arnoldi_opts &o, const ArnoldiAug *aug,
                bool force_lanczos) {
  ks_finish_tail(ks);
  int herm = o.ishermitian;
  if (herm < 0) herm = op.ishermitian;
  const bool lanczos = force_lanczos || herm != 0;
  return dispatch_dtype(ks.dtypeT, [&](auto tag) {
    using T = typename decltype(tag)::type;
    return arnoldi_T<T>(ks, op, (const T *)b_dev, o, aug, lanczos);
  });
}

template <class TC> static inline TC coef_as(const std::vector<double> &cbuf, size_t k, bool cplx_buf);
template <> inline double coef_as<double>(const std::vector<double> &b, size_t k, bool c) { return c ? b[2 * k] : b[k]; }
template <> inline float coef_as<float>(const std::vector<double> &b, size_t k, bool c) { return (float)(c ? b[2 * k] : b[k]); }
template <> inline cplx coef_as<cplx>(const std::vector<double> &b, size_t k, bool c) { return c ? make_cplx(b[2 * k], b[2 * k + 1]) : make_cplx(b[k], 0.0); }
template <> inline cplx32 coef_as<cplx32>(const std::vector<double> &b, size_t k, bool c) {
  return c ? make_cplx32((float)b[2 * k], (float)b[2 * k + 1]) : make_cplx32((float)b[k], 0.0f);
}

template <class TV, class TC>
static void combine_launch(Ks &ks, Ctx *c, int mcols, int ncols, const std::vector<double> &cbuf, bool cplx_buf, double scale, void *Wd,
                           int64_t ldwd, int64_t rows, bool by_value, const LcSpec *lc, const int32_t *rowmap = nullptr) {
  const int mc = std::max(mcols, 0);
  const TV *V = ks.V.as<TV>();
  if (by_value) {
    dev::CoefVec<TC> cv;
    for (int i = 0; i < mc; ++i) cv.c[i] = coef_as<TC>(cbuf, (size_t)i, cplx_buf);
    if (lc) {
      if constexpr (std::is_same<TV, TC>::value) {
        dev::LcTerms<TC> lt{};
        lt.nterms = lc->nterms;
        lt.pscale = lc->pscale;
        for (int l = 0; l < lc->nterms; ++l) { lt.in[l] = reinterpret_cast<const TC *>(lc->in[l]); lt.coef[l] = ST<TC>::from_real(lc->coef[l]); }
        dev::combine1_lc<TV, TC>(c->stream, rows, V, ks.ldv, mc, cv, scale, lt, (TC *)Wd);
      }
    } else {
      dev::combine1<TV, TC>(c->stream, rows, V, ks.ldv, mc, cv, scale, (TC *)Wd, rowmap);
    }
    return;
  }
  if (ncols >= 2 && ncols <= dev::COEF_MAT_COLS && mc >= 1 && (size_t)mc * ncols <= (size_t)dev::COEF_MAT_MAX) {
    dev::CoefMat<TC> cm;
    for (size_t k = 0; k < (size_t)mc * ncols; ++k) cm.c[k] = coef_as<TC>(cbuf, k, cplx_buf);
    dev::combine_v<TV, TC>(c->stream, rows, V, ks.ldv, mc, cm, ncols, scale, (TC *)Wd, ldwd);
    return;
  }
  std::vector<TC> ch((size_t)mcols * ncols);
  for (size_t k = 0; k < ch.size(); ++k) ch[k] = coef_as<TC>(cbuf, k, cplx_buf);
  DevBuf cdev(ch.size() * sizeof(TC) + 16);
  HIPCHECK(hipMemcpyAsync(cdev.p, ch.data(), ch.size() * sizeof(TC), hipMemcpyHostToDevice, c->stream));
  dev::combine<TV, TC>(c->stream, rows, V, ks.ldv, mc, cdev.as<TC>(), mcols, ncols, scale, (TC *)Wd, ldwd);
  HIPCHECK(hipStreamSynchronize(c->stream));
}

void combine_host_coef(Ks &ks, int mcols, int ncols, const void *coef_host, int ldc, int coef_dtype, double scale,
                       void *W, int64_t ldw, int w_loc, int w_dtype, const LcSpec *lc) {
  Ctx *c = ks.ctx;
  c->use();
  if (mcols < 0 || mcols > ks.maxiter + 1) fail(EXPV_MI_ASSERTION, "combine: more columns than the basis holds");
  const bool Tc = dtype_is_complex(ks.dtypeT);
  const bool Cc = dtype_is_complex(coef_dtype) || Tc || dtype_is_complex(w_dtype);
  if (Cc && !dtype_is_complex(w_dtype)) fail(EXPV_MI_ARGUMENT_ERROR, "InexactError: complex result into a real output");
  if (dtype_is_32bit(ks.dtypeT) != dtype_is_32bit(w_dtype))
    fail(EXPV_MI_ARGUMENT_ERROR, "combine: the output must have the precision of the basis (32-bit basis -> Float32 / ComplexF32 result)");
  const int64_t rows = ks.n;
  const size_t wsz = dtype_size(w_dtype);
  std::vector<double> cbuf((size_t)mcols * ncols * (Cc ? 2 : 1));
  for (int q = 0; q < ncols; ++q)
    for (int i = 0; i < mcols; ++i) {
      double re, im = 0.0;
      if (coef_dtype == EXPV_MI_C64) {
        const double *p = reinterpret_cast<const double *>(coef_host) + 2 * ((size_t)q * ldc + i);
        re = p[0];
        im = p[1];
      } else {
        re = reinterpret_cast<const double *>(coef_host)[(size_t)q * ldc + i];
      }
      if (Cc) {
        cbuf[2 * ((size_t)q * mcols + i)] = re;
        cbuf[2 * ((size_t)q * mcols + i) + 1] = im;
      } else {
        cbuf[(size_t)q * mcols + i] = re;
      }
    }
  if (ks.scale_pending) {
    for (int q = 0; q < ncols; ++q)
      for (int i = 0; i < mcols && i < ks.scale_cols; ++i) {
        const double sc = ks.colscale_host[i];
        if (Cc) { cbuf[2 * ((size_t)q * mcols + i)] *= sc; cbuf[2 * ((size_t)q * mcols + i) + 1] *= sc; }
        else cbuf[(size_t)q * mcols + i] *= sc;
// ... 26 lines not shown
      else if (!Tc) combine_launch<float, cplx32>(ks, c, mcols, ncols, cbuf, Cc, scale, Wd, ldwd, rows, by_value, lc, rowmap);
      else combine_launch<cplx32, cplx32>(ks, c, mcols, ncols, cbuf, Cc, scale, Wd, ldwd, rows, by_value, lc, rowmap);
    }
  }
  if (unperm && !fuse_out) permute_out(c, *ks.vperm, Wd, ldwd, W, w_loc, ldw, ncols, wsz);
  else if (w_loc == EXPV_MI_HOST) copy_out_2d(c, W, EXPV_MI_HOST, ldw, Wd, ldwd, rows, ncols, wsz);
  else if (!c->async_out) HIPCHECK(hipStreamSynchronize(c->stream));
}

static void zero_output(Ctx *c, void *W, int64_t ldw, int w_loc, int64_t rows, int ncols, size_t esz) {
  for (int q = 0; q < ncols; ++q) {
    char *col = reinterpret_cast<char *>(W) + (size_t)q * ldw * esz;
    if (w_loc == EXPV_MI_HOST) std::memset(col, 0, (size_t)rows * esz);
    else HIPCHECK(hipMemsetAsync(col, 0, (size_t)rows * esz, c->stream));
  }
  if (w_loc != EXPV_MI_HOST && !c->async_out) HIPCHECK(hipStreamSynchronize(c->stream));
}

void expv_eval(Ks &ks, double t_re, double t_im, void *w, int w_loc, int w_dtype) {
  const int m = ks.m;
  const bool tc = (t_im != 0.0);
  if ((tc || dtype_is_complex(ks.dtypeT)) && !dtype_is_complex(w_dtype))
    fail(EXPV_MI_ARGUMENT_ERROR, "expv!: w must be complex when t or the basis is complex");
  if (ks.beta == 0.0) {
    zero_output(ks.ctx, w, ks.n, w_loc, ks.n, 1, dtype_size(w_dtype));
    return;
  }
  Mat<cd> Hc(m, m);
  for (int j = 0; j < m; ++j)
    for (int i = 0; i < m; ++i) Hc(i, j) = getH(ks, i, j);
  bool herm = true, offreal = true;
  for (int j = 0; j < m && herm; ++j)
    for (int i = 0; i < m; ++i)
      if (Hc(i, j) != std::conj(Hc(j, i))) { herm = false; break; }
  for (int i = 0; i + 1 < m; ++i)
    if (Hc(i, i + 1).imag() != 0.0) offreal = false;
  const cd t(t_re, t_im);
  if (herm && offreal) {
    std::vector<double> d(m), e(m > 1 ? m - 1 : 0);
    for (int i = 0; i < m; ++i) d[i] = Hc(i, i).real();
    for (int i = 0; i + 1 < m; ++i) e[i] = Hc(i, i + 1).real();
    if (tc) {
      std::vector<cd> coef = dense::symtridiag_expcol<cd>(d, e, t);
      combine_host_coef(ks, m, 1, coef.data(), m, EXPV_MI_C64, ks.beta, w, ks.n, w_loc, w_dtype);
    } else {
      std::vector<double> coef = dense::symtridiag_expcol<double>(d, e, t_re);
      combine_host_coef(ks, m, 1, coef.data(), m, EXPV_MI_F64, ks.beta, w, ks.n, w_loc, w_dtype);
    }
    return;
  }
  const bool cplx_small = tc || dtype_is_complex(ks.dtypeU);
  if (cplx_small) {
    for (auto &v : Hc.a) v *= t;
    dense::expm_higham2005base(Hc);
    combine_host_coef(ks, m, 1, Hc.data(), m, EXPV_MI_C64, ks.beta, w, ks.n, w_loc, w_dtype);
  } else {
    Mat<double> Hr(m, m);
    for (size_t i = 0; i < Hr.a.size(); ++i) Hr.a[i] = Hc.a[i].real() * t_re;
    ht_mark(7);
    dense::expm_higham2005base(Hr);
    ht_mark(5);
    combine_host_coef(ks, m, 1, Hr.data(), m, EXPV_MI_F64, ks.beta, w, ks.n, w_loc, w_dtype);
    ht_mark(6);
  }
}

void phiv_coefficients(Ks &ks, double t_re, double t_im, int k, int correct, std::vector<double> &Ce_out, int *mext_out,
                       bool *is_cplx, double *errest) {
  const int m = ks.m;
  const bool tc = (t_im != 0.0);
  if (k < 1) fail(EXPV_MI_ARGUMENT_ERROR, "phiv!: k >= 1 required");
  const cd t(t_re, t_im);
  const int hend_r = m, hend_c = m - 1 + (ks.augmented != 0 ? 1 : 0);
  const bool cplx_small = tc || dtype_is_complex(ks.dtypeU);
  const int mext = m + (correct ? 1 : 0);
  double err = 0.0;
  if (cplx_small) {
    Mat<cd> Hc(m, m);
    for (int j = 0; j < m; ++j)
      for (int i = 0; i < m; ++i) Hc(i, j) = getH(ks, i, j) * t;
    std::vector<cd> e(m, cd(0));
    if (m > 0) e[0] = cd(1);
    Mat<cd> C2 = dense::phiv_dense(Hc, e, k);
    ks_finish_tail(ks);
    const cd hend = getH(ks, hend_r, hend_c);
    Mat<cd> Ce(mext, k + 1);
    for (int q = 0; q <= k; ++q)
      for (int i = 0; i < m; ++i) Ce(i, q) = C2(i, q);
    if (correct)
      for (int i = 1; i <= k; ++i) Ce(m, i - 1) = hend * t * C2(m - 1, i);
    err = std::abs(ks.beta * hend * t * C2(m - 1, k));
    Ce_out.resize((size_t)2 * mext * (k + 1));
    std::memcpy(Ce_out.data(), Ce.data(), sizeof(double) * Ce_out.size());
  } else {
    Mat<double> Hr(m, m);
    for (int j = 0; j < m; ++j)
      for (int i = 0; i < m; ++i) Hr(i, j) = getH(ks, i, j).real() * t_re;
    std::vector<double> e(m, 0.0);
    if (m > 0) e[0] = 1.0;
    Mat<double> C2 = dense::phiv_dense(Hr, e, k);
    ks_finish_tail(ks);
    const cd hend = getH(ks, hend_r, hend_c);
    Mat<double> Ce(mext, k + 1);
    for (int q = 0; q <= k; ++q)
      for (int i = 0; i < m; ++i) Ce(i, q) = C2(i, q);
    if (correct)
      for (int i = 1; i <= k; ++i) Ce(m, i - 1) = hend.real() * t_re * C2(m - 1, i);
    err = std::fabs(ks.beta * hend.real() * t_re * C2(m - 1, k));
    Ce_out.assign(Ce.data(), Ce.data() + (size_t)mext * (k + 1));
  }
  *mext_out = mext;
  *is_cplx = cplx_small;
  if (errest) *errest = err;
}

// ... 176 lines not shown
```

### exponentialutilities.jl_amd/csrc/host_dense.h

```cpp
#pragma once
#include <algorithm>
#include <cmath>
#include <complex>
#include <cstring>
#include <limits>
#include <stdexcept>
#include <type_traits>
#include <vector>
#if defined(__AVX2__) && defined(__FMA__)
#include <immintrin.h>
#endif

namespace expv_mi {
namespace dense {

using cd = std::complex<double>;
using cf = std::complex<float>;
template <class S> struct real_of { typedef S type; };
template <class R> struct real_of<std::complex<R>> { typedef R type; };
template <class S> using real_t = typename real_of<S>::type;

struct SingularError : std::runtime_error {
  SingularError() : std::runtime_error("SingularException(0): Pade denominator is singular") {}
};
// ... 122 lines not shown
    const __m256d xv = _mm256_loadu_pd(x + 2 * i);
    const __m256d t = _mm256_fmaddsub_pd(xv, ar, _mm256_mul_pd(_mm256_permute_pd(xv, 0x5), ai));
    _mm256_storeu_pd(y + 2 * i, _mm256_sub_pd(_mm256_loadu_pd(y + 2 * i), t));
  }
  for (; i < n; ++i) yc[i] -= xc[i] * alpha;
}
#endif

template <class S>
inline void matmul(Mat<S> &C, const Mat<S> &A, const Mat<S> &B) {
  const int n = A.r, k = A.c, m = B.c;
#if defined(__AVX2__) && defined(__FMA__)
  if constexpr (std::is_same<S, double>::value) {
    if (C.r != n || C.c != m) C = Mat<S>(n, m);
    matmul_f64(C.a.data(), A.a.data(), B.a.data(), n, k, m);
    return;
  }
  if constexpr (std::is_same<S, std::complex<double>>::value) {
    if (C.r != n || C.c != m) C = Mat<S>(n, m);
    matmul_c64(C.a.data(), A.a.data(), B.a.data(), n, k, m);
    return;
  }
#endif
  if (C.r != n || C.c != m) C = Mat<S>(n, m);
  else std::fill(C.a.begin(), C.a.end(), S(0));
  int j = 0;
  for (; j + 4 <= m; j += 4) {
    S *__restrict__ c0 = &C.a[(size_t)j * n];
    S *__restrict__ c1 = c0 + n;
    S *__restrict__ c2 = c1 + n;
    S *__restrict__ c3 = c2 + n;
    for (int l = 0; l < k; ++l) {
      const S b0 = B(l, j), b1 = B(l, j + 1), b2 = B(l, j + 2), b3 = B(l, j + 3);
      if (!nonzero(b0) && !nonzero(b1) && !nonzero(b2) && !nonzero(b3)) continue;
      const S *__restrict__ ac = &A.a[(size_t)l * n];
      for (int i = 0; i < n; ++i) {
        const S a = ac[i];
        c0[i] += a * b0;
        c1[i] += a * b1;
        c2[i] += a * b2;
        c3[i] += a * b3;
      }
    }
  }
  for (; j < m; ++j)
    for (int l = 0; l < k; ++l) {
      const S b = B(l, j);
      if (!nonzero(b)) continue;
      const S *__restrict__ ac = &A.a[(size_t)l * n];
      S *__restrict__ cc = &C.a[(size_t)j * n];
      for (int i = 0; i < n; ++i) cc[i] += ac[i] * b;
    }
}

template <class S>
inline real_t<S> opnorm1(const Mat<S> &A) {
  real_t<S> best = 0;
  for (int j = 0; j < A.c; ++j) {
    real_t<S> s = 0;
    for (int i = 0; i < A.r; ++i)
      if (nonzero(A(i, j))) s += absv(A(i, j));
    best = std::max(best, s);
  }
  return best;
}

template <class S>
inline double opnorm1_raw(const S *H, int ld, int r, int c) {
  double best = 0;
  for (int j = 0; j < c; ++j) {
    double s = 0;
    for (int i = 0; i < r; ++i) s += absv(H[(size_t)j * ld + i]);
    best = std::max(best, s);
  }
  return best;
}

template <class S>
struct Balance {
  int ilo = 1, ihi = 0;
  std::vector<real_t<S>> scale;
};

inline double re_of(double x) { return x; }
inline double im_of(double) { return 0.0; }
inline float re_of(float x) { return x; }
inline float im_of(float) { return 0.0f; }
template <class R> inline R re_of(const std::complex<R> &x) { return x.real(); }
template <class R> inline R im_of(const std::complex<R> &x) { return x.imag(); }

template <class S>
inline real_t<S> nrm2_strided(const S *x, int n, int inc) {
  typedef real_t<S> R;
  R ss = 0;
  for (int i = 0; i < n; ++i) {
    const S v = x[(size_t)i * inc];
    ss += re_of(v) * re_of(v) + im_of(v) * im_of(v);
  }
  const R lo = sizeof(R) == 8 ? R(1e-280) : R(1e-30f), hi = sizeof(R) == 8 ? R(1e280) : R(1e30f);
  if (ss > lo && ss < hi) return std::sqrt(ss);
  R scale = 0, ssq = 1;
  for (int i = 0; i < n; ++i) {
    const S v = x[(size_t)i * inc];
    const R parts[2] = {re_of(v), im_of(v)};
    for (R p : parts) {
      if (p != 0) {
// ... 197 lines not shown
#if defined(__AVX2__) && defined(__FMA__)
      if constexpr (std::is_same<S, std::complex<double>>::value) { caxpy_sub_c64(mj + k + 1, mk + k + 1, mkj, n - k - 1); continue; }
#endif
      for (int i = k + 1; i < n; ++i) mj[i] -= mk[i] * mkj;
    }
  }
#if defined(__AVX2__) && defined(__FMA__)
  if constexpr (std::is_same<S, double>::value) {
    trsolve_f64(M.a.data(), n, X.a.data(), nrhs);
    return;
  }
#endif
  std::vector<S> Xt((size_t)n * nrhs);
  for (int j = 0; j < nrhs; ++j)
    for (int i = 0; i < n; ++i) Xt[(size_t)i * nrhs + j] = X.a[(size_t)j * n + i];
  for (int k = 0; k < n; ++k) {
    const S *__restrict__ rk = &Xt[(size_t)k * nrhs];
    const S *__restrict__ mk = &M.a[(size_t)k * n];
    for (int i = k + 1; i < n; ++i) {
      const S l = mk[i];
      if (!nonzero(l)) continue;
      S *__restrict__ ri = &Xt[(size_t)i * nrhs];
#if defined(__AVX2__) && defined(__FMA__)
      if constexpr (std::is_same<S, std::complex<double>>::value) { caxpy_sub_c64(ri, rk, l, nrhs); continue; }
#endif
      for (int j = 0; j < nrhs; ++j) ri[j] -= l * rk[j];
    }
  }
  for (int k = n - 1; k >= 0; --k) {
    S *__restrict__ rk = &Xt[(size_t)k * nrhs];
    const S *__restrict__ mk = &M.a[(size_t)k * n];
    const S d = mk[k];
    if constexpr (std::is_same<S, std::complex<double>>::value) {
      const S dinv = S(1) / d;
      for (int j = 0; j < nrhs; ++j) rk[j] *= dinv;
    } else {
      for (int j = 0; j < nrhs; ++j) rk[j] /= d;
    }
    for (int i = 0; i < k; ++i) {
      const S u = mk[i];
      if (!nonzero(u)) continue;
      S *__restrict__ ri = &Xt[(size_t)i * nrhs];
#if defined(__AVX2__) && defined(__FMA__)
      if constexpr (std::is_same<S, std::complex<double>>::value) { caxpy_sub_c64(ri, rk, u, nrhs); continue; }
#endif
      for (int j = 0; j < nrhs; ++j) ri[j] -= u * rk[j];
    }
  }
  for (int j = 0; j < nrhs; ++j)
    for (int i = 0; i < n; ++i) X.a[(size_t)j * n + i] = Xt[(size_t)i * nrhs + j];
}

template <class S>
inline Mat<S> pade_evaluate(const Mat<S> &A, const double *C, int N) {
  const int n = A.r;
  Mat<S> A2, P(n, n), U(n, n), V(n, n), tmp;
  matmul(A2, A, A);
  typedef real_t<S> R;
  for (int i = 0; i < n; ++i) { P(i, i) = S(1); U(i, i) = S(R(C[1])); V(i, i) = S(R(C[0])); }
  for (int k = 1; k <= N / 2 - 1; ++k) {
    const int k2 = 2 * k;
    if (k == 1) {
      P = A2;
    } else {
      matmul(tmp, P, A2);
      std::swap(P.a, tmp.a);
    }
    const S cu = S(R(C[k2 + 1])), cv = S(R(C[k2]));
    for (size_t i = 0; i < P.a.size(); ++i) { U.a[i] += cu * P.a[i]; V.a[i] += cv * P.a[i]; }
  }
  matmul(tmp, A, U);
  std::swap(U.a, tmp.a);
  Mat<S> X(n, n), D(n, n);
  for (size_t i = 0; i < X.a.size(); ++i) { X.a[i] = V.a[i] + U.a[i]; D.a[i] = V.a[i] - U.a[i]; }
  lu_solve(D, X);
  return X;
}

static const double PADE_C3[] = {120.0, 60.0, 12.0, 1.0};
static const double PADE_C5[] = {30240.0, 15120.0, 3360.0, 420.0, 30.0, 1.0};
static const double PADE_C7[] = {17297280.0, 8648640.0, 1995840.0, 277200.0, 25200.0, 1512.0, 56.0, 1.0};
static const double PADE_C9[] = {17643225600.0, 8821612800.0, 2075673600.0, 302702400.0, 30270240.0,
                                 2162160.0,     110880.0,     3960.0,       90.0,        1.0};
static const double PADE_C13[] = {64764752532480000.0, 32382376266240000.0, 7771770303897600.0,
                                  1187353796428800.0,  129060195264000.0,   10559470521600.0,
                                  670442572800.0,      33522128640.0,       1323241920.0,
                                  40840800.0,          960960.0,            16380.0,
                                  182.0,               1.0};

template <class S>
inline void expm_higham2005base(Mat<S> &A) {
  typedef real_t<S> R;
  const int n = A.r;
  if (n == 0) return;
  for (const auto &v : A.a)
    if (!std::isfinite(re_of(v)) || !std::isfinite(im_of(v)))
      throw std::invalid_argument("ArgumentError: matrix contains Infs or NaNs");
  Balance<S> bal = gebal(A);
  const R nA = opnorm1(A);
  Mat<S> X;
  if (nA <= R(2.1)) {
    if (nA > R(0.95)) X = pade_evaluate(A, PADE_C9, 10);
    else if (nA > R(0.25)) X = pade_evaluate(A, PADE_C7, 8);
    else if (nA > R(0.015)) X = pade_evaluate(A, PADE_C5, 6);
    else X = pade_evaluate(A, PADE_C3, 4);
  } else {
    const R s = std::log2(nA / R(5.4));
    int si = 0;
    if (s > 0) {
      si = (int)std::ceil(s);
      const R sc = std::ldexp(R(1), si);
      for (auto &v : A.a) v /= sc;
    }
    X = pade_evaluate(A, PADE_C13, 14);
    if (s > 0) {
      Mat<S> tmp;
      for (int t = 0; t < si; ++t) { matmul(tmp, X, X); std::swap(X.a, tmp.a); }
    }
  }
  unbalance(X, bal);
  A = X;
}

template <bool ENDS_ONLY = false>
inline void symtridiag_eig(std::vector<double> &d, std::vector<double> e_in, Mat<double> &Z) {
  const int n = (int)d.size();
  const int zr = ENDS_ONLY ? 2 : n;
  Z = Mat<double>(zr, n);
  if (ENDS_ONLY) {
    if (n > 0) { Z(0, 0) = 1.0; Z(1, n - 1) = 1.0; }
  } else {
    for (int i = 0; i < n; ++i) Z(i, i) = 1.0;
  }
  if (n <= 1) return;
  std::vector<double> e(n, 0.0);
  for (int i = 0; i + 1 < n; ++i) e[i] = e_in[i];
  for (int l = 0; l < n; ++l) {
    int iter = 0, m;
    do {
      for (m = l; m + 1 < n; ++m) {
        const double dd = std::fabs(d[m]) + std::fabs(d[m + 1]);
        if (std::fabs(e[m]) <= 2.220446049250313e-16 * dd) break;
      }
      if (m != l) {
        if (++iter > 200) throw std::runtime_error("symtridiag_eig: no convergence");
        double g = (d[l + 1] - d[l]) / (2.0 * e[l]);
        double r = std::hypot(g, 1.0);
        g = d[m] - d[l] + e[l] / (g + (g >= 0 ? std::fabs(r) : -std::fabs(r)));
        double s = 1.0, c = 1.0, p = 0.0;
        int i;
        for (i = m - 1; i >= l; --i) {
          double f = s * e[i], b = c * e[i];
          r = std::hypot(f, g);
          e[i + 1] = r;
          if (r == 0.0) { d[i + 1] -= p; e[m] = 0.0; break; }
          s = f / r;
          c = g / r;
          g = d[i + 1] - p;
          r = std::fma(2.0 * c, b, (d[i] - g) * s);
          p = s * r;
          {
#pragma clang fp contract(off)
            d[i + 1] = g + p;
          }
          g = std::fma(c, r, -b);
          for (int k = 0; k < zr; ++k) {
            f = Z(k, i + 1);
            const double zk = Z(k, i);
            Z(k, i + 1) = std::fma(c, f, s * zk);
            Z(k, i) = std::fma(c, zk, -(s * f));
          }
        }
        if (r == 0.0 && i >= l) continue;
        d[l] -= p;
// ... 64 lines not shown
```

### exponentialutilities.jl_amd/csrc/kernels.h

```cpp
#pragma once
#include "device_types.h"

namespace expv_mi {
namespace dev {

constexpr int BLOCK = 256;
constexpr int GROUP_SIZE = 64;
constexpr int MAX_GROUPS = 32;
constexpr int MAX_GRID = GROUP_SIZE * MAX_GROUPS;
constexpr int MAX_RED_VALUES = 4 * 64;
constexpr int LOWSYNC_MAX = 64;

enum DotsMode { DOTS_STRICT = 0, DOTS_LOWSYNC = 1, DOTS_LANCZOS = 2 };

struct BatchStrides {
  int64_t V, ybuf, part, gpart, Hdev, gram, hcoef, Aval, st;
};

template <class T>
struct DotsArgs {
  const T *V; int64_t ldv; int64_t n;
  const T *y;
  const T *x;
  int c0, dir, nd;
// ... 259 lines not shown
constexpr int PL_MAX_M = 128;
struct LanczosPlArgs {
  const double *dia_val; int64_t dia_ld; int ndiag; int dia_off[PIPE_DIA_MAX]; int w;
  int64_t n_dia;
  double *V; int64_t ldv; int64_t n;
  const double *u0;
  double *part;
  uint32_t *count;
  uint32_t *flags;
  double *out;
  int m, want_tail; double tol; int spin_limit;
};
bool lanczos_pl(hipStream_t s, const LanczosPlArgs &a);
int lanczos_pl_capacity();
bool pipe_resident(hipStream_t s, const ResArgs &ra);
int pipe_resident_capacity();
void pipe_step(hipStream_t s, const PipeArgsT<double> &pa, int nbatch = 1, int batch_rounds = 2);
void pipe_step(hipStream_t s, const PipeArgsT<cplx> &pa, int nbatch = 1, int batch_rounds = 2);
void pipe_step(hipStream_t s, const PipeArgsT<float> &pa, int nbatch = 1, int batch_rounds = 2);
void pipe_step(hipStream_t s, const PipeArgsT<cplx32> &pa, int nbatch = 1, int batch_rounds = 2);
bool pipe_step_wave(hipStream_t s, const PipeArgs &pa, int64_t max_abs_off);
int pipe_step_wave_live(hipStream_t s, const PipeArgs &pa, int64_t max_abs_off);
bool pipe_step_wave(hipStream_t s, const PipeArgsT<float> &pa, int64_t max_abs_off);
int pipe_step_wave_live(hipStream_t s, const PipeArgsT<float> &pa, int64_t max_abs_off);
int pipe_step_ring(hipStream_t s, const PipeArgsT<double> &pa, bool live);
int pipe_step_ring(hipStream_t s, const PipeArgsT<float> &pa, bool live);
int pipe_step_ring(hipStream_t s, const PipeArgsT<cplx> &pa, bool live);
int pipe_step_ring(hipStream_t s, const PipeArgsT<cplx32> &pa, bool live);
int pipe_step_live(hipStream_t s, const PipeArgsT<double> &pa);
int pipe_step_live(hipStream_t s, const PipeArgsT<cplx> &pa);
int pipe_step_live(hipStream_t s, const PipeArgsT<float> &pa);
int pipe_step_live(hipStream_t s, const PipeArgsT<cplx32> &pa);
template <class T> constexpr int pipe_max_window() { return ST<T>::is_complex ? PIPE_CH_CPLX - 1 : PIPE_CH - 1; }
void pipe_gate(hipStream_t s, const uint32_t *arrive, int expected, StepState *st, int spin_limit);
constexpr int PIPE_FLAG_COPIES = 16, PIPE_FLAG_STRIDE = 1024;
constexpr int PIPE_ARRIVE_STRIDE = 32;
constexpr int PIPE_ARRIVE_STEP = PIPE_FLAG_COPIES * PIPE_ARRIVE_STRIDE;
constexpr uint32_t PIPE_SEQ_MASK = 0xfffffu;
template <class T> void scale_columns(hipStream_t s, T *V, int64_t ldv, int64_t n, const double *scales, int ncols);

template <class T> void dots(hipStream_t s, const DotsArgs<T> &a);
template <class T> void update(hipStream_t s, const UpdateArgs<T> &a);

template <class TV, class TC>
void combine(hipStream_t s, int64_t n, const TV *V, int64_t ldv, int m, const TC *C, int ldc, int ncols,
             double scale, TC *W, int64_t ldw);

constexpr int COEF_BY_VALUE_MAX = 64;
template <class TC> struct CoefVec { TC c[COEF_BY_VALUE_MAX]; };
constexpr int COEF_MAT_MAX = 192, COEF_MAT_COLS = 6;
template <class TC> struct CoefMat { TC c[COEF_MAT_MAX]; };
template <class TV, class TC>
void combine_v(hipStream_t s, int64_t n, const TV *V, int64_t ldv, int m, const CoefMat<TC> &cm, int ncols, double scale, TC *W, int64_t ldw);
template <class TV, class TC>
void combine1(hipStream_t s, int64_t n, const TV *V, int64_t ldv, int m, const CoefVec<TC> &cv, double scale, TC *W,
              const int32_t *rowmap = nullptr);
template <class TC> struct LcTerms { int nterms; const TC *in[6]; TC coef[6]; double pscale; };
template <class TV, class TC>
void combine1_lc(hipStream_t s, int64_t n, const TV *V, int64_t ldv, int m, const CoefVec<TC> &cv, double scale, const LcTerms<TC> &lt, TC *W);

template <class T>
struct LincombArgs { T *out; const T *in[8]; T coef[8]; int nterms; int64_t n; };
template <class T> void lincomb(hipStream_t s, const LincombArgs<T> &a);

void widen_real_to_complex(hipStream_t s, cplx *dst, const double *src, int64_t n);

}
}
```

### exponentialutilities.jl_amd/csrc/kernels.hip

```cpp
#include <stdexcept>
#include <string>
#include <cstdint>
#include <map>
#include <mutex>

#include <type_traits>

#include "kernel_common.h"

namespace expv_mi {
namespace dev {

int device_cus() {
  static int cus = [] {
    int d = 0, v = 256;
    (void)hipGetDevice(&d);
    if (hipDeviceGetAttribute(&v, hipDeviceAttributeMultiprocessorCount, d) != hipSuccess || v <= 0) v = 256;
    return v;
  }();
  return cus;
}
int resident_blocks(const void *kernel) {
  static std::mutex mu;
  static std::map<const void *, int> cache;
// ... 720 lines not shown
  TC *cs = reinterpret_cast<TC *>(smem);
  for (int e = threadIdx.x; e < m * NC; e += BLOCK) cs[e] = cm.c[(e / NC) + (e % NC) * m];
  __syncthreads();
  combine_body<TV, TC, NC>(n, V, ldv, m, cs, scale, W, ldw);
}
template <class TV, class TC, int NC>
__device__ __forceinline__ void combine_body(int64_t n, const TV *__restrict__ V, int64_t ldv, int m, const TC *cs, double scale,
                                             TC *__restrict__ W, int64_t ldw) {
  constexpr int N = Pack<TV>::N;
  const bool al = ((ldv * sizeof(TV)) % 16 == 0) && is_al16(V);
  const int64_t tile = (int64_t)BLOCK * N;
  for (int64_t base = (int64_t)blockIdx.x * tile; base < n; base += (int64_t)gridDim.x * tile) {
    const int64_t i = base + (int64_t)threadIdx.x * N;
    if (i >= n) break;
    TC acc[N][NC];
#pragma unroll
    for (int k = 0; k < N; ++k)
#pragma unroll
      for (int q = 0; q < NC; ++q) acc[k][q] = ST<TC>::zero();
    int c = 0;
    for (; c + 8 <= m; c += 8) {
      Pack<TV> vv[8];
#pragma unroll
      for (int u = 0; u < 8; ++u) vv[u] = ld_pack(V + (int64_t)(c + u) * ldv, i, n, al);
#pragma unroll
      for (int u = 0; u < 8; ++u)
#pragma unroll
        for (int q = 0; q < NC; ++q) {
          const TC cq = cs[(c + u) * NC + q];
#pragma unroll
          for (int k = 0; k < N; ++k) mulacc<TV, TC>(acc[k][q], vv[u].v[k], cq);
        }
    }
    for (; c < m; ++c) {
      const Pack<TV> vv = ld_pack(V + (int64_t)c * ldv, i, n, al);
#pragma unroll
      for (int q = 0; q < NC; ++q) {
        const TC cq = cs[c * NC + q];
#pragma unroll
        for (int k = 0; k < N; ++k) mulacc<TV, TC>(acc[k][q], vv.v[k], cq);
      }
    }
#pragma unroll
    for (int k = 0; k < N; ++k)
      if (i + k < n) {
#pragma unroll
        for (int q = 0; q < NC; ++q) W[(i + k) + (int64_t)q * ldw] = ST<TC>::mul_real(acc[k][q], scale);
      }
  }
}
template <class TV, class TC>
__global__ __launch_bounds__(BLOCK) void k_combine1(int64_t n, const TV *__restrict__ V, int64_t ldv, int m,
                                                    CoefVec<TC> cv, double scale, TC *__restrict__ W, int64_t rpb,
                                                    const int32_t *__restrict__ rowmap) {
  constexpr int N = Pack<TV>::N;
  const bool al = ((ldv * sizeof(TV)) % 16 == 0) && is_al16(V);
  const int64_t r0 = (int64_t)blockIdx.x * rpb, r1 = (r0 + rpb < n) ? r0 + rpb : n;
  for (int64_t i = r0 + (int64_t)threadIdx.x * N; i < r1; i += (int64_t)BLOCK * N) {
    TC acc[N];
#pragma unroll
    for (int k = 0; k < N; ++k) acc[k] = ST<TC>::zero();
    int c = 0;
    for (; c + 8 <= m; c += 8) {
      Pack<TV> vv[8];
#pragma unroll
      for (int u = 0; u < 8; ++u) vv[u] = ld_pack(V + (int64_t)(c + u) * ldv, i, n, al);
#pragma unroll
      for (int u = 0; u < 8; ++u)
#pragma unroll
        for (int k = 0; k < N; ++k) mulacc<TV, TC>(acc[k], vv[u].v[k], cv.c[c + u]);
    }
    for (; c < m; ++c) {
      const Pack<TV> vv = ld_pack(V + (int64_t)c * ldv, i, n, al);
#pragma unroll
      for (int k = 0; k < N; ++k) mulacc<TV, TC>(acc[k], vv.v[k], cv.c[c]);
    }
#pragma unroll
    for (int k = 0; k < N; ++k)
      if (i + k < n) W[rowmap ? (int64_t)rowmap[i + k] : i + k] = ST<TC>::mul_real(acc[k], scale);
  }
}
template <class TV, class TC>
void combine1(hipStream_t s, int64_t n, const TV *V, int64_t ldv, int m, const CoefVec<TC> &cv, double scale, TC *W, const int32_t *rowmap) {
  const RowPlan p = plan_rows(n, 64 * Pack<TV>::N, resident_blocks((const void *)k_combine1<TV, TC>));
  hipLaunchKernelGGL((k_combine1<TV, TC>), dim3(p.nblocks), dim3(BLOCK), 0, s, n, V, ldv, m, cv, scale, W,
                     p.rows_per_block, rowmap);
}

template <class TV, class TC>
__global__ __launch_bounds__(BLOCK) void k_combine1_lc(int64_t n, const TV *__restrict__ V, int64_t ldv, int m, CoefVec<TC> cv,
                                                       double scale, LcTerms<TC> lt, TC *__restrict__ W, int64_t rpb) {
  constexpr int N = Pack<TV>::N;
  const bool al = ((ldv * sizeof(TV)) % 16 == 0) && is_al16(V);
  const int64_t r0 = (int64_t)blockIdx.x * rpb, r1 = (r0 + rpb < n) ? r0 + rpb : n;
  for (int64_t i = r0 + (int64_t)threadIdx.x * N; i < r1; i += (int64_t)BLOCK * N) {
    TC acc[N];
#pragma unroll
    for (int k = 0; k < N; ++k) acc[k] = ST<TC>::zero();
    int c = 0;
    for (; c + 8 <= m; c += 8) {
      Pack<TV> vv[8];
#pragma unroll
      for (int u = 0; u < 8; ++u) vv[u] = ld_pack(V + (int64_t)(c + u) * ldv, i, n, al);
#pragma unroll
      for (int u = 0; u < 8; ++u)
#pragma unroll
        for (int k = 0; k < N; ++k) mulacc<TV, TC>(acc[k], vv[u].v[k], cv.c[c + u]);
    }
    for (; c < m; ++c) {
      const Pack<TV> vv = ld_pack(V + (int64_t)c * ldv, i, n, al);
#pragma unroll
      for (int k = 0; k < N; ++k) mulacc<TV, TC>(acc[k], vv.v[k], cv.c[c]);
    }
#pragma unroll
    for (int k = 0; k < N; ++k) {
      if (i + k >= n) continue;
      TC v = ST<TC>::mul_real(ST<TC>::mul_real(acc[k], scale), lt.pscale);
      for (int l = 0; l < lt.nterms; ++l) ST<TC>::fma_(v, lt.coef[l], lt.in[l][i + k]);
      W[i + k] = v;
    }
  }
}
template <class TV, class TC>
void combine1_lc(hipStream_t s, int64_t n, const TV *V, int64_t ldv, int m, const CoefVec<TC> &cv, double scale, const LcTerms<TC> &lt, TC *W) {
  const RowPlan p = plan_rows(n, 64 * Pack<TV>::N, resident_blocks((const void *)k_combine1_lc<TV, TC>));
  hipLaunchKernelGGL((k_combine1_lc<TV, TC>), dim3(p.nblocks), dim3(BLOCK), 0, s, n, V, ldv, m, cv, scale, lt, W, p.rows_per_block);
}

template <class TV, class TC>
void combine_v(hipStream_t s, int64_t n, const TV *V, int64_t ldv, int m, const CoefMat<TC> &cm, int ncols, double scale, TC *W, int64_t ldw) {
  const int g = grid_for(n, BLOCK * Pack<TV>::N * 2);
  const size_t sh = (size_t)m * ncols * sizeof(TC);
  switch (ncols) {
    case 6: hipLaunchKernelGGL((k_combine_v<TV, TC, 6>), dim3(g), dim3(BLOCK), sh, s, n, V, ldv, m, cm, scale, W, ldw); break;
    case 5: hipLaunchKernelGGL((k_combine_v<TV, TC, 5>), dim3(g), dim3(BLOCK), sh, s, n, V, ldv, m, cm, scale, W, ldw); break;
    case 4: hipLaunchKernelGGL((k_combine_v<TV, TC, 4>), dim3(g), dim3(BLOCK), sh, s, n, V, ldv, m, cm, scale, W, ldw); break;
    case 3: hipLaunchKernelGGL((k_combine_v<TV, TC, 3>), dim3(g), dim3(BLOCK), sh, s, n, V, ldv, m, cm, scale, W, ldw); break;
    default: hipLaunchKernelGGL((k_combine_v<TV, TC, 2>), dim3(g), dim3(BLOCK), sh, s, n, V, ldv, m, cm, scale, W, ldw); break;
  }
// ... 29 lines not shown
  const int64_t tile = (int64_t)BLOCK * N;
  for (int64_t base = (int64_t)blockIdx.x * tile; base < a.n; base += (int64_t)gridDim.x * tile) {
    const int64_t i = base + (int64_t)threadIdx.x * N;
    if (i >= a.n) break;
    Pack<T> acc;
#pragma unroll
    for (int k = 0; k < N; ++k) acc.v[k] = ST<T>::zero();
    for (int t = 0; t < a.nterms; ++t) {
      const Pack<T> v = ld_pack_user(a.in[t], i, a.n, al);
#pragma unroll
      for (int k = 0; k < N; ++k) {
        if (t == 0) acc.v[k] = ST<T>::mul(a.coef[0], v.v[k]);
        else ST<T>::fma_(acc.v[k], a.coef[t], v.v[k]);
      }
    }
    st_pack_user(a.out, i, a.n, al, acc);
  }
}
template <class T>
void lincomb(hipStream_t s, const LincombArgs<T> &a) {
  const int g = grid_for(a.n, BLOCK * Pack<T>::N * 2);
  hipLaunchKernelGGL(k_lincomb<T>, dim3(g), dim3(BLOCK), 0, s, a);
}

__global__ __launch_bounds__(BLOCK) void k_widen(cplx *__restrict__ dst, const double *__restrict__ src, int64_t n) {
  for (int64_t i = (int64_t)blockIdx.x * BLOCK + threadIdx.x; i < n; i += (int64_t)gridDim.x * BLOCK)
    dst[i] = make_cplx(src[i], 0.0);
}
void widen_real_to_complex(hipStream_t s, cplx *dst, const double *src, int64_t n) {
  hipLaunchKernelGGL(k_widen, dim3(grid_for(n, BLOCK * 4)), dim3(BLOCK), 0, s, dst, src, n);
}

#define INST(T)                                                                                                    \
  template void sumsq<T>(hipStream_t, const T *, int64_t, double *, double *, StepState *);                        \
  template void scale_copy<T>(hipStream_t, T *, const T *, int64_t, double, int);                                  \
  template void scale_by_state<T>(hipStream_t, T *, int64_t, const StepState *, int);                              \
  template void fill_zero<T>(hipStream_t, T *, int64_t);                                                           \
  template void spmv_ovf<T>(hipStream_t, const OvfView<T> &, const T *, const StepState *, int, int64_t, int, bool);      \
  template void gemv_dense<T>(hipStream_t, int64_t, const T *, int64_t, const T *, T *, T *, int,                  \
                              const StepState *, int, int64_t);                                                                \
  template void aug_apply<T>(hipStream_t, int64_t, int, const T *, int64_t, const T *, T *, const StepState *,     \
                             int);                                                                                 \
  template void dots<T>(hipStream_t, const DotsArgs<T> &);                                                         \
  template void update<T>(hipStream_t, const UpdateArgs<T> &);                                                     \
  template void lincomb<T>(hipStream_t, const LincombArgs<T> &);
INST(double)
INST(cplx)
INST(float)
INST(cplx32)
template void combine1_lc<float, float>(hipStream_t, int64_t, const float *, int64_t, int, const CoefVec<float> &, double,
                                        const LcTerms<float> &, float *);
template void combine1_lc<cplx32, cplx32>(hipStream_t, int64_t, const cplx32 *, int64_t, int, const CoefVec<cplx32> &, double,
                                          const LcTerms<cplx32> &, cplx32 *);
template void combine1<float, float>(hipStream_t, int64_t, const float *, int64_t, int, const CoefVec<float> &, double, float *, const int32_t *);
template void combine1<float, cplx32>(hipStream_t, int64_t, const float *, int64_t, int, const CoefVec<cplx32> &, double, cplx32 *, const int32_t *);
template void combine1<cplx32, cplx32>(hipStream_t, int64_t, const cplx32 *, int64_t, int, const CoefVec<cplx32> &, double, cplx32 *, const int32_t *);
template void combine_v<float, float>(hipStream_t, int64_t, const float *, int64_t, int, const CoefMat<float> &, int, double, float *, int64_t);
template void combine_v<float, cplx32>(hipStream_t, int64_t, const float *, int64_t, int, const CoefMat<cplx32> &, int, double, cplx32 *, int64_t);
template void combine_v<cplx32, cplx32>(hipStream_t, int64_t, const cplx32 *, int64_t, int, const CoefMat<cplx32> &, int, double, cplx32 *, int64_t);
template void combine_v<double, double>(hipStream_t, int64_t, const double *, int64_t, int, const CoefMat<double> &, int, double, double *, int64_t);
template void combine_v<double, cplx>(hipStream_t, int64_t, const double *, int64_t, int, const CoefMat<cplx> &, int, double, cplx *, int64_t);
template void combine_v<cplx, cplx>(hipStream_t, int64_t, const cplx *, int64_t, int, const CoefMat<cplx> &, int, double, cplx *, int64_t);
template void combine<float, float>(hipStream_t, int64_t, const float *, int64_t, int, const float *, int, int, double, float *, int64_t);
template void combine<float, cplx32>(hipStream_t, int64_t, const float *, int64_t, int, const cplx32 *, int, int, double, cplx32 *, int64_t);
template void combine<cplx32, cplx32>(hipStream_t, int64_t, const cplx32 *, int64_t, int, const cplx32 *, int, int, double, cplx32 *, int64_t);
template void combine1_lc<double, double>(hipStream_t, int64_t, const double *, int64_t, int, const CoefVec<double> &, double,
                                          const LcTerms<double> &, double *);
template void combine1_lc<cplx, cplx>(hipStream_t, int64_t, const cplx *, int64_t, int, const CoefVec<cplx> &, double,
                                      const LcTerms<cplx> &, cplx *);
template void combine1<double, double>(hipStream_t, int64_t, const double *, int64_t, int, const CoefVec<double> &,
                                       double, double *, const int32_t *);
template void combine1<double, cplx>(hipStream_t, int64_t, const double *, int64_t, int, const CoefVec<cplx> &, double,
                                     cplx *, const int32_t *);
template void combine1<cplx, cplx>(hipStream_t, int64_t, const cplx *, int64_t, int, const CoefVec<cplx> &, double,
                                   cplx *, const int32_t *);
template void combine<double, double>(hipStream_t, int64_t, const double *, int64_t, int, const double *, int, int,
                                      double, double *, int64_t);
template void combine<double, cplx>(hipStream_t, int64_t, const double *, int64_t, int, const cplx *, int, int, double,
                                    cplx *, int64_t);
template void combine<cplx, cplx>(hipStream_t, int64_t, const cplx *, int64_t, int, const cplx *, int, int, double,
                                  cplx *, int64_t);


template <int K>
__device__ __forceinline__ void ref_halve(double (&a)[K], int lane) {
  int half = K / 2, off = 32;
  for (; half >= 1; half >>= 1, off >>= 1) {
    const bool hi = (lane & off) != 0;
    for (int i = 0; i < half; ++i) {
      const double send = hi ? a[i] : a[i + half];
      const double keep = hi ? a[i + half] : a[i];
      a[i] = keep + __shfl_xor(send, off, 64);
    }
  }
  for (; off >= 1; off >>= 1) a[0] += __shfl_xor(a[0], off, 64);
}
template <int K>
__device__ __forceinline__ int selftest_multi(const double *in, int lane, int tid) {
  double a[K], b[K];
#pragma unroll
  for (int k = 0; k < K; ++k) a[k] = b[k] = in[(size_t)k * BLOCK + tid];
  wave_reduce_multi<K>(a);
  ref_halve<K>(b, lane);
  return __double_as_longlong(a[0]) != __double_as_longlong(b[0]);
}
__global__ __launch_bounds__(BLOCK) void k_selftest_lanes(const double *in, unsigned long long *out) {
  const int tid = threadIdx.x, lane = tid & 63;
  const double v = in[tid];
  int bad0 = 0;
  bad0 += __double_as_longlong(xor_sum<32>(v)) != __double_as_longlong(v + __shfl_xor(v, 32, 64));
  bad0 += __double_as_longlong(xor_sum<16>(v)) != __double_as_longlong(v + __shfl_xor(v, 16, 64));
  bad0 += __double_as_longlong(xor_sum<8>(v)) != __double_as_longlong(v + __shfl_xor(v, 8, 64));
  bad0 += __double_as_longlong(xor_sum<4>(v)) != __double_as_longlong(v + __shfl_xor(v, 4, 64));
  bad0 += __double_as_longlong(xor_sum<2>(v)) != __double_as_longlong(v + __shfl_xor(v, 2, 64));
  bad0 += __double_as_longlong(xor_sum<1>(v)) != __double_as_longlong(v + __shfl_xor(v, 1, 64));
  double r = v, q = v;
  for (int o = 32; o >= 1; o >>= 1) r += __shfl_xor(r, o, 64);
  for (int o = 32; o > 0; o >>= 1) q += __shfl_down(q, o, 64);
  const int bad1 = __double_as_longlong(xor_reduce<32>(v)) != __double_as_longlong(r);
  double r16 = v;
  for (int o = 16; o >= 1; o >>= 1) r16 += __shfl_xor(r16, o, 64);
  const int bad2 = __double_as_longlong(xor_reduce<16>(v)) != __double_as_longlong(r16);
  const double ws = wave_sum(v);
  const int bad3 = (lane == 0) && __double_as_longlong(ws) != __double_as_longlong(q);
  const int bad4 = selftest_multi<16>(in, lane, tid) + selftest_multi<8>(in + 16 * BLOCK, lane, tid) +
                   selftest_multi<2>(in + 24 * BLOCK, lane, tid) + selftest_multi<4>(in + 26 * BLOCK, lane, tid);
  const int bad5 = selftest_multi<32>(in, lane, tid);
  if (bad0) atomicAdd(out + 0, (unsigned long long)bad0);
// ... 157 lines not shown
```

### include/expv_mi.h

```cpp
#ifndef EXPV_MI_H
#define EXPV_MI_H

#include <stddef.h>
#include <stdint.h>

#ifdef __cplusplus
extern "C" {
#endif

typedef struct expv_mi_ctx_s *expv_mi_ctx_t;
typedef struct expv_mi_op_s *expv_mi_op_t;
typedef struct expv_mi_ks_s *expv_mi_ks_t;
typedef struct expv_mi_comm_s *expv_mi_comm_t;
typedef struct expv_mi_tscache_s *expv_mi_tscache_t;

typedef enum {
  EXPV_MI_OK = 0,
  EXPV_MI_DIMENSION_MISMATCH = 1,
  EXPV_MI_ARGUMENT_ERROR = 2,
  EXPV_MI_ASSERTION = 3,
  EXPV_MI_SINGULAR = 4,
  EXPV_MI_UNSUPPORTED = 5,
  EXPV_MI_OUT_OF_MEMORY = 6,
  EXPV_MI_HIP_ERROR = 7,
  EXPV_MI_BOUNDS = 8
} expv_mi_status;

typedef enum { EXPV_MI_F64 = 0, EXPV_MI_C64 = 1, EXPV_MI_F32 = 2, EXPV_MI_C32 = 3 } expv_mi_dtype;
typedef enum { EXPV_MI_HOST = 0, EXPV_MI_DEVICE = 1 } expv_mi_loc;

typedef enum { EXPV_MI_ORTHO_AUTO = 0, EXPV_MI_ORTHO_MGS = 1, EXPV_MI_ORTHO_LOWSYNC = 2,
               EXPV_MI_ORTHO_PIPELINED = 3 } expv_mi_ortho;

int expv_mi_ctx_create(int device_id, void *stream, expv_mi_ctx_t *ctx);
int expv_mi_ctx_destroy(expv_mi_ctx_t ctx);
int expv_mi_ctx_sync(expv_mi_ctx_t ctx);
int expv_mi_ctx_set_async_outputs(expv_mi_ctx_t ctx, int on);
int expv_mi_ctx_set_pipeline_overlap(expv_mi_ctx_t ctx, int on);
int expv_mi_ctx_set_option(expv_mi_ctx_t ctx, const char *name, int64_t value);
int expv_mi_ctx_get_option(expv_mi_ctx_t ctx, const char *name, int64_t *value);
int expv_mi_ctx_counters(expv_mi_ctx_t ctx, int64_t out[8]);
int expv_mi_ctx_selftest(expv_mi_ctx_t ctx, int64_t out[8]);
enum {
  EXPV_MI_PATH_MODULAR = 1, EXPV_MI_PATH_TWO_KERNEL = 2, EXPV_MI_PATH_PIPELINE = 4, EXPV_MI_PATH_WAVE = 8,
  EXPV_MI_PATH_OVERLAPPED = 16, EXPV_MI_PATH_REDO_SERIAL = 32, EXPV_MI_PATH_REDO_WAVE_OFF = 64,
  EXPV_MI_PATH_RESIDENT = 128,
  EXPV_MI_PATH_PATCH = 256,
  EXPV_MI_PATH_PIPELINED_LANCZOS = 512,
  EXPV_MI_PATH_FA2_PIPELINED = 1024
};
const char *expv_mi_last_error(expv_mi_ctx_t ctx);
const char *expv_mi_version(void);

int expv_mi_malloc(expv_mi_ctx_t ctx, size_t bytes, void **dptr);
int expv_mi_free(expv_mi_ctx_t ctx, void *dptr);
int expv_mi_memcpy_h2d(expv_mi_ctx_t ctx, void *dst, const void *src, size_t bytes);
int expv_mi_memcpy_d2h(expv_mi_ctx_t ctx, void *dst, const void *src, size_t bytes);

enum {
  EXPV_MI_K_FIRSTSTEP = 0, EXPV_MI_K_MATVEC = 1, EXPV_MI_K_DOTS = 2, EXPV_MI_K_UPDATE = 3,
  EXPV_MI_K_SCALE = 4, EXPV_MI_K_COMBINE = 5, EXPV_MI_K_FUSED_A = 6, EXPV_MI_K_FUSED_B = 7,
  EXPV_MI_K_LINCOMB = 8, EXPV_MI_K_AUG = 9, EXPV_MI_K_BATCH = 10, EXPV_MI_K_COUNT = 11
};
int expv_mi_prof_enable(expv_mi_ctx_t ctx, int on);
int expv_mi_prof_reset(expv_mi_ctx_t ctx);
int expv_mi_prof_get(expv_mi_ctx_t ctx, int kernel_id, int64_t *launches, double *total_ms);
const char *expv_mi_prof_name(int kernel_id);


int expv_mi_op_create_csc(expv_mi_ctx_t ctx, int dtype, int64_t n, const int64_t *colptr,
                          const int64_t *rowval, const void *nzval, int index_base, expv_mi_op_t *op);
int expv_mi_op_create_csr(expv_mi_ctx_t ctx, int dtype, int64_t n, const void *rowptr, const void *colind,
                          const void *vals, int idx_bytes, int index_base, expv_mi_op_t *op);
int expv_mi_op_create_csr_loc(expv_mi_ctx_t ctx, int dtype, int64_t n, int64_t nnz, const void *rowptr, const void *colind,
                              const void *vals, int idx_bytes, int index_base, int loc, expv_mi_op_t *op);
int expv_mi_op_create_csc_loc(expv_mi_ctx_t ctx, int dtype, int64_t n, int64_t nnz, const void *colptr, const void *rowval,
                              const void *nzval, int idx_bytes, int index_base, int loc, expv_mi_op_t *op);
int expv_mi_op_create_coo_loc(expv_mi_ctx_t ctx, int dtype, int64_t n, int64_t nnz, const void *row, const void *col, const void *vals,
                              int idx_bytes, int index_base, int loc, expv_mi_op_t *op);
int expv_mi_op_ingest_info(expv_mi_op_t op, int64_t out[8]);
int expv_mi_op_create_dense(expv_mi_ctx_t ctx, int dtype, int64_t n, const void *A, int64_t lda, int loc,
                            expv_mi_op_t *op);
typedef int (*expv_mi_matvec_fn)(void *user, const void *x_dev, void *y_dev, void *hip_stream);
int expv_mi_op_create_callback(expv_mi_ctx_t ctx, int dtype, int64_t n, expv_mi_matvec_fn fn, void *user,
                               int ishermitian, int64_t nnz_hint, expv_mi_op_t *op);
int expv_mi_op_update_values(expv_mi_op_t op, const void *vals, int loc);
int expv_mi_op_destroy(expv_mi_op_t op);
int expv_mi_op_info(expv_mi_op_t op, int64_t *n, int64_t *nnz, int *ishermitian, double *opnorm_inf,
                    int *dtype);
int expv_mi_op_reorder_info(expv_mi_op_t op, int64_t out[4]);
int expv_mi_op_patch_info(expv_mi_op_t op, int64_t out[8]);
int expv_mi_plan_cache(int what, int64_t value, int64_t out[4]);
int expv_mi_host_patch_order(int64_t n, const int32_t *rowptr, const int32_t *colind, int dtype, int32_t *perm, int32_t *ring_count,
                             int64_t out[8]);
// ... 91 lines not shown
typedef struct {
  int32_t num_timesteps;
  int32_t matvecs;
  int32_t m_final;
  int32_t arnoldi_calls;
  int32_t arnoldi_reused;
  int32_t stalled_steps;
} expv_mi_timestep_stats;
void expv_mi_timestep_opts_default(expv_mi_timestep_opts *o);
int expv_mi_timestep_caches_create(expv_mi_ctx_t ctx, int dtype, int64_t n, int maxiter, int p,
                                   expv_mi_tscache_t *cache);
int expv_mi_timestep_caches_destroy(expv_mi_tscache_t cache);
int expv_mi_phiv_timestep(expv_mi_ctx_t ctx, expv_mi_op_t op, int nts, double *ts, const void *B,
                          int64_t ldb, int ncoef, int b_loc, void *U, int64_t ldu, int u_loc,
                          const expv_mi_timestep_opts *opts, expv_mi_tscache_t caches,
                          expv_mi_timestep_stats *stats);

typedef struct {
  int32_t mmin, mmax, m, iop, ishermitian, task1, ortho, reserved;
  double tol;
} expv_mi_kiops_opts;
void expv_mi_kiops_opts_default(expv_mi_kiops_opts *o);
int expv_mi_kiops(expv_mi_ctx_t ctx, expv_mi_op_t op, const double *tau_out, int ntau, int tau_ncols,
                  const void *u, int64_t ldu, int ncols_u, int u_loc, void *w, int64_t ldw, int w_loc,
                  const expv_mi_kiops_opts *opts, int64_t stats[5]);

int expv_mi_expv_batch(expv_mi_ctx_t ctx, int dtype, int64_t n, int nprob, const int32_t *rowptr,
                       const int32_t *colind, const void *vals, int64_t nnz_per_prob, int mat_loc,
                       const double *t, const void *b, int64_t ldb, int b_loc, void *w, int64_t ldw,
                       int w_loc, const expv_mi_arnoldi_opts *opts, int32_t *m_used);

int expv_mi_expv_batch_multi(expv_mi_ctx_t *ctxs, int nctx, int dtype, int64_t n, int nprob, const int32_t *rowptr,
                             const int32_t *colind, const void *vals, int64_t nnz_per_prob, const double *t,
                             const void *b, int64_t ldb, void *w, int64_t ldw, int w_loc,
                             const expv_mi_arnoldi_opts *opts, int32_t *m_used);

int expv_mi_rccl_available(void);
int expv_mi_rccl_unique_id(void *id128);
int expv_mi_comm_create(expv_mi_ctx_t ctx, const void *id128, int nranks, int rank, expv_mi_comm_t *comm);
int expv_mi_gather_rccl(expv_mi_comm_t comm, const void *send_dev, void *recv_dev, int64_t count, int dtype);
int expv_mi_comm_destroy(expv_mi_comm_t comm);

enum {
  EXPV_MI_ABI_ARNOLDI_OPTS = 0, EXPV_MI_ABI_EXPV_STATS = 1, EXPV_MI_ABI_TIMESTEP_OPTS = 2,
  EXPV_MI_ABI_TIMESTEP_STATS = 3, EXPV_MI_ABI_KIOPS_OPTS = 4, EXPV_MI_ABI_COUNT = 5
};
size_t expv_mi_abi_sizeof(int kind);
const char *expv_mi_abi_layout(int kind);

int expv_mi_host_pattern_info(int64_t n, const int32_t *rowptr, const int32_t *colind, int dtype, int64_t out[8]);
int expv_mi_host_rcm(int64_t n, const int32_t *rowptr, const int32_t *colind, int dtype, int32_t *perm, int64_t out[4]);
int expv_mi_host_wrapsum(const void *buf, uint64_t nbytes, uint64_t out[2]);
int expv_mi_host_expm(int dtype, int n, void *A, int lda);
int expv_mi_host_gebal(int dtype, int n, void *A, int lda, int64_t *ilo, int64_t *ihi, double *scale);
int expv_mi_host_symtridiag_expcol(int n, const double *d, const double *e, double t_re, double t_im,
                                   double *out_c64);
int expv_mi_host_symtridiag_exp_last(int n, const double *d, const double *e, double t_re, double t_im,
                                     double *out_c64);
int expv_mi_host_phiv_dense(int dtype, int m, int k, const void *A, int lda, const void *v, void *w);

#ifdef __cplusplus
}
#endif
#endif
```

Baseline: 27140 matvecs/s.

## Compute only first column of small exp(H) and fold state reset into combine

The host-side dense exponential of the Hessenberg matrix now computes only column 0 of exp(tH). When no squaring is needed it solves for one column, and otherwise the final squaring becomes a single matrix-vector product. Work buffers are reused across calls. The device zeroing of the step-state and H buffers is folded into the final combine kernel of the previous call, so the next fresh Arnoldi can skip a separate zeroing launch. Zeroing of host H is also deferred until after the step launches are enqueued. This cuts host latency and one launch per expv call, at the cost of extra cross-call state flags that must stay correctly invalidated.

New measurement: 27400 matvecs/s, median of 6. Within noise of the previous version (+0.9%).

```diff
diff --git a/exponentialutilities.jl_amd/_lib.py b/exponentialutilities.jl_amd/_lib.py
--- a/exponentialutilities.jl_amd/_lib.py
+++ b/exponentialutilities.jl_amd/_lib.py
@@ -64,6 +64,7 @@
     "expv_mi_ctx_set_async_outputs": (_i, [_vp, _i]),
     "expv_mi_ctx_set_pipeline_overlap": (_i, [_vp, _i]),
     "expv_mi_ctx_counters": (_i, [_vp, _pi64]),
+    "expv_mi_ctx_counters_more": (_i, [_vp, _pi64]),
     "expv_mi_ctx_selftest": (_i, [_vp, _pi64]),
     "expv_mi_ctx_set_option": (_i, [_vp, C.c_char_p, _i64]),
     "expv_mi_ctx_get_option": (_i, [_vp, C.c_char_p, _pi64]),
@@ -140,6 +141,7 @@
     "expv_mi_host_rcm": (_i, [C.c_int64, _vp, _vp, _i, _vp, _vp]),
     "expv_mi_host_wrapsum": (_i, [_vp, C.c_uint64, _vp]),
     "expv_mi_host_expm": (_i, [_i, _i, _vp, _i]),
+    "expv_mi_host_expm_col0": (_i, [_i, _i, _vp, _i, _vp]),
     "expv_mi_host_gebal": (_i, [_i, _i, _vp, _i, _vp, _vp, _vp]),
     "expv_mi_host_symtridiag_expcol": (_i, [_i, _pd, _pd, _d, _d, _pd]),
     "expv_mi_host_symtridiag_exp_last": (_i, [_i, _pd, _pd, _d, _d, _pd]),
diff --git a/exponentialutilities.jl_amd/api.py b/exponentialutilities.jl_amd/api.py
--- a/exponentialutilities.jl_amd/api.py
+++ b/exponentialutilities.jl_amd/api.py
@@ -10,7 +10,7 @@
 __all__ = [
     "Context", "default_context", "MIOperator", "DeviceArray", "KrylovSubspace", "arnoldi", "arnoldi_",
     "lanczos_", "expv", "expv_", "phiv", "phiv_", "expv_timestep", "expv_timestep_", "phiv_timestep",
-    "phiv_timestep_", "kiops", "timestep_caches", "expv_batch", "expv_batch_multi", "RcclComm", "rccl_available", "rccl_unique_id", "ExpvMIError", "DimensionMismatch", "host_expm",
+    "phiv_timestep_", "kiops", "timestep_caches", "expv_batch", "expv_batch_multi", "RcclComm", "rccl_available", "rccl_unique_id", "ExpvMIError", "DimensionMismatch", "host_expm", "host_expm_col0",
     "exponential", "exponential_", "mul_", "phi", "phi_", "balance_", "host_gebal",
     "host_phiv_dense", "host_symtridiag_expcol", "host_symtridiag_exp_last", "host_pattern_info", "host_rcm", "host_patch_order", "clear_operator_cache", "plan_cache",
 ]
@@ -82,11 +82,16 @@
         _check(L.load().expv_mi_ctx_selftest(self._h, out), self._h)
         return tuple(int(x) for x in out)
 
-    def counters(self):
+    def counters(self, extended=False):
         out = (C.c_int64 * 8)()
         _check(L.load().expv_mi_ctx_counters(self._h, out), self._h)
         keys = ("krylov_steps", "factorisations", "pipeline", "overlapped", "redo_serial", "redo_wave_off", "op_applies", "h_by_copy")
-        return dict(zip(keys, (int(v) for v in out)))
+        d = dict(zip(keys, (int(v) for v in out)))
+        if extended:
+            more = (C.c_int64 * 8)()
+            _check(L.load().expv_mi_ctx_counters_more(self._h, more), self._h)
+            d["head_resets"] = int(more[0])
+        return d
 
     def set_pipeline_overlap(self, on=True):
         _check(L.load().expv_mi_ctx_set_pipeline_overlap(self._h, int(bool(on))), self._h)
@@ -1550,6 +1555,14 @@
     return A
 
 
+def host_expm_col0(A):
+    A = np.array(A, dtype=_host_dtype(np.asarray(A).dtype), order="F", copy=True)
+    n = A.shape[0]
+    col = np.empty(n, dtype=A.dtype)
+    _check(L.load().expv_mi_host_expm_col0(_HOST_CODES[A.dtype], n, A.ctypes.data, max(n, 1), col.ctypes.data))
+    return col
+
+
 def host_gebal(A):
     A = np.array(A, dtype=_host_dtype(np.asarray(A).dtype), order="F", copy=True)
     if A.ndim != 2 or A.shape[0] != A.shape[1]:
diff --git a/exponentialutilities.jl_amd/csrc/capi.hip b/exponentialutilities.jl_amd/csrc/capi.hip
--- a/exponentialutilities.jl_amd/csrc/capi.hip
+++ b/exponentialutilities.jl_amd/csrc/capi.hip
@@ -1186,6 +1186,14 @@
     for (int i = 0; i < n; ++i) reinterpret_cast<S *>(A)[(size_t)j * lda + i] = M(i, j);
 }
 template <class S>
+void host_expm_col0_T(int n, const void *A, int lda, void *col) {
+  Mat<S> M(n, n);
+  for (int j = 0; j < n; ++j)
+    for (int i = 0; i < n; ++i) M(i, j) = reinterpret_cast<const S *>(A)[(size_t)j * lda + i];
+  dense::ExpmWork<S> w;
+  dense::expm_higham2005base_col0(M, reinterpret_cast<S *>(col), w);
+}
+template <class S>
 void host_gebal_T(int n, void *A, int lda, int64_t *ilo, int64_t *ihi, double *scale) {
   Mat<S> M(n, n);
   for (int j = 0; j < n; ++j)
@@ -1354,6 +1362,12 @@
   if (!ctx || !out) return EXPV_MI_ARGUMENT_ERROR;
   out[0] = ctx->cnt_steps; out[1] = ctx->cnt_fact; out[2] = ctx->cnt_pipe; out[3] = ctx->cnt_live;
   out[4] = ctx->cnt_serial_redo; out[5] = ctx->cnt_wave_redo; out[6] = ctx->cnt_opapply; out[7] = ctx->cnt_copy;
+  return EXPV_MI_OK;
+}
+int expv_mi_ctx_counters_more(expv_mi_ctx_t ctx, int64_t out[8]) {
+  if (!ctx || !out) return EXPV_MI_ARGUMENT_ERROR;
+  for (int i = 0; i < 8; ++i) out[i] = 0;
+  out[0] = ctx->cnt_head_reset;
   return EXPV_MI_OK;
 }
 int expv_mi_ctx_selftest(expv_mi_ctx_t ctx, int64_t out[8]) {
@@ -2541,6 +2555,18 @@
       case EXPV_MI_F32: host_expm_T<float>(n, A, lda); break;
       case EXPV_MI_C32: host_expm_T<dense::cf>(n, A, lda); break;
       default: fail(EXPV_MI_ARGUMENT_ERROR, "host_expm: unknown dtype");
+    }
+  });
+}
+int expv_mi_host_expm_col0(int dtype, int n, const void *A, int lda, void *col) {
+  return guarded(nullptr, [&] {
+    if (n < 0 || lda < n || (n > 0 && (!A || !col))) fail(EXPV_MI_ARGUMENT_ERROR, "host_expm_col0: bad n / lda / A / col");
+    switch (dtype) {
+      case EXPV_MI_F64: host_expm_col0_T<double>(n, A, lda, col); break;
+      case EXPV_MI_C64: host_expm_col0_T<cd>(n, A, lda, col); break;
+      case EXPV_MI_F32: host_expm_col0_T<float>(n, A, lda, col); break;
+      case EXPV_MI_C32: host_expm_col0_T<dense::cf>(n, A, lda, col); break;
+      default: fail(EXPV_MI_ARGUMENT_ERROR, "host_expm_col0: unknown dtype");
     }
   });
 }
diff --git a/exponentialutilities.jl_amd/csrc/engine.h b/exponentialutilities.jl_amd/csrc/engine.h
--- a/exponentialutilities.jl_amd/csrc/engine.h
+++ b/exponentialutilities.jl_amd/csrc/engine.h
@@ -132,6 +132,7 @@
   int dense_force_singular = 0;
   int dense_tile = 0;
   int64_t cnt_steps = 0, cnt_fact = 0, cnt_live = 0, cnt_serial_redo = 0, cnt_wave_redo = 0, cnt_opapply = 0, cnt_pipe = 0, cnt_copy = 0;
+  int64_t cnt_head_reset = 0;
   int last_path = 0;
   hipStream_t stream2 = nullptr;
   hipEvent_t ev_fork = nullptr, ev_join = nullptr;
@@ -344,6 +345,9 @@
   std::vector<double> colscale_host;
   bool scale_pending = false;
   bool skip_tail = false;
+  bool state_clean = false, reset_wanted = false;
+  dense::ExpmWork<double> expw_real;
+  dense::ExpmWork<dense::cd> expw_cplx;
   int scale_cols = 0;
   DevBuf ubuf, ybuf;
   DevBuf extbuf;
diff --git a/exponentialutilities.jl_amd/csrc/engine_core.hip b/exponentialutilities.jl_amd/csrc/engine_core.hip
--- a/exponentialutilities.jl_amd/csrc/engine_core.hip
+++ b/exponentialutilities.jl_amd/csrc/engine_core.hip
@@ -168,6 +168,8 @@
   ks.scale_pending = false;
   ks.scale_cols = 0;
   ks.skip_tail = false;
+  ks.state_clean = false;
+  ks.reset_wanted = false;
   ks.defer_tail_req = false;
   ks.pipe_closed = false;
   ks.mbox_armed = false;
@@ -180,6 +182,8 @@
 
 void ks_resize(Ks &ks, int maxiter) {
   ks.ctx->use();
+  ks.state_clean = false;
+  ks.reset_wanted = false;
   ks_materialize(ks);
   const bool isaug = ks.augmented != 0;
   const size_t esz = dtype_size(ks.dtypeT), usz = dtype_size(ks.dtypeU);
@@ -433,7 +437,9 @@
   StepState *st = nullptr;
   double *part = nullptr, *gpart = nullptr;
   bool h_zeroed = false;
+  bool host_h_stale = false;
   bool fa2_pl_used = false;
+  bool state_was_clean = false;
   bool cont_reset_done = false;
   bool tail_deferred = false;
   bool use_fused = false, single_red = false, use_pipe = false, use_wave = false, use_ring = false, mbox_generic = false;
@@ -462,6 +468,9 @@
     hview_cols = m + (isaug ? 1 : 0);
 
     choose_step_form();
+    state_was_clean = ks.state_clean && fresh && use_pipe;
+    ks.state_clean = false;
+    ks.reset_wanted = false;
     if (ks.b_natural) {
       ks.b_natural = false;
       b_nat = true;
@@ -481,11 +490,11 @@
       }
     }
     if (fresh) first_step();
-    if (ks.beta == 0.0) return 0;
+    if (ks.beta == 0.0) { zero_host_h(); return 0; }
     iop = o.iop;
     if (iop == 0) iop = m;
     jstart = (lanczos && !ks.lanczos_continue) ? 1 : init;
-    if (jstart > m) return 0;
+    if (jstart > m) { zero_host_h(); return 0; }
     ct_mark("  arnoldi!: form chosen, first step set up");
     reset_device_state();
     ct_mark("  arnoldi!: device state reset enqueued");
@@ -497,6 +506,7 @@
     else if (use_fused) steps_two_kernel_two_reductions();
     else steps_modular();
     ct_mark("  arnoldi!: all step launches enqueued");
+    zero_host_h();
     return read_back();
   }
 
@@ -615,10 +625,19 @@
   }
   }
 
-  void first_step() {
+  void zero_host_h() {
+    if (!host_h_stale) return;
+    host_h_stale = false;
     for (int j = 0; j < hview_cols; ++j)
       std::memset(&ks.H[(size_t)j * ks.ldh * dtype_size(ks.dtypeU)], 0, (size_t)hview_rows * dtype_size(ks.dtypeU));
-    dev::zero_two(s, st, ks.state.bytes, ks.Hdev.as<T>() + (size_t)(jstart - 1) * ks.ldhd, sizeof(T) * (size_t)ks.ldhd * (m - jstart + 1));
+  }
+  void first_step() {
+    host_h_stale = true;
+    if (!use_pipe) zero_host_h();
+    if (!state_was_clean) {
+      dev::zero_two(s, st, ks.state.bytes, ks.Hdev.as<T>() + (size_t)(jstart - 1) * ks.ldhd, sizeof(T) * (size_t)ks.ldhd * (m - jstart + 1));
+      ++c->cnt_head_reset;
+    }
     h_zeroed = true;
     double extra = 0.0;
     const T *src = b;
@@ -1151,6 +1170,7 @@
     c->last_path |= EXPV_MI_PATH_REDO_SERIAL;
     return r;
   }
+  ks.reset_wanted = from_mbox && ks.skip_tail && use_pipe && ks.pipe_live_used && !ks.pipe_resident_used && !tail_deferred && !mbox_generic;
   if (use_fused && fresh) {
     ks.beta = std::sqrt(h.beta0sq);
     if (ks.beta == 0.0) { ks.gram_rows = 0; return 0; }
@@ -1285,7 +1305,9 @@
         dev::combine1_lc<TV, TC>(c->stream, rows, V, ks.ldv, mc, cv, scale, lt, (TC *)Wd);
       }
     } else {
-      dev::combine1<TV, TC>(c->stream, rows, V, ks.ldv, mc, cv, scale, (TC *)Wd, rowmap);
+      dev::ZeroTwo zt{ks.state.as<unsigned long long>(), ks.state.bytes / 8, ks.Hdev.as<unsigned long long>(), ks.Hdev.bytes / 8};
+      dev::combine1<TV, TC>(c->stream, rows, V, ks.ldv, mc, cv, scale, (TC *)Wd, rowmap, ks.reset_wanted ? &zt : nullptr);
+      if (ks.reset_wanted) { ks.reset_wanted = false; ks.state_clean = true; }
     }
     return;
   }
@@ -1418,15 +1440,17 @@
   const bool cplx_small = tc || dtype_is_complex(ks.dtypeU);
   if (cplx_small) {
     for (auto &v : Hc.a) v *= t;
-    dense::expm_higham2005base(Hc);
-    combine_host_coef(ks, m, 1, Hc.data(), m, EXPV_MI_C64, ks.beta, w, ks.n, w_loc, w_dtype);
+    std::vector<cd> col(m);
+    dense::expm_higham2005base_col0(Hc, col.data(), ks.expw_cplx);
+    combine_host_coef(ks, m, 1, col.data(), m, EXPV_MI_C64, ks.beta, w, ks.n, w_loc, w_dtype);
   } else {
     Mat<double> Hr(m, m);
     for (size_t i = 0; i < Hr.a.size(); ++i) Hr.a[i] = Hc.a[i].real() * t_re;
     ht_mark(7);
-    dense::expm_higham2005base(Hr);
+    std::vector<double> col(m);
+    dense::expm_higham2005base_col0(Hr, col.data(), ks.expw_real);
     ht_mark(5);
-    combine_host_coef(ks, m, 1, Hr.data(), m, EXPV_MI_F64, ks.beta, w, ks.n, w_loc, w_dtype);
+    combine_host_coef(ks, m, 1, col.data(), m, EXPV_MI_F64, ks.beta, w, ks.n, w_loc, w_dtype);
     ht_mark(6);
   }
 }
diff --git a/exponentialutilities.jl_amd/csrc/host_dense.h b/exponentialutilities.jl_amd/csrc/host_dense.h
--- a/exponentialutilities.jl_amd/csrc/host_dense.h
+++ b/exponentialutilities.jl_amd/csrc/host_dense.h
@@ -198,6 +198,30 @@
       for (int i = 0; i < n; ++i) cc[i] += ac[i] * b;
     }
 }
+
+#if defined(__AVX2__) && defined(__FMA__)
+inline void matmul_col0(double *c, const Mat<double> &A, const Mat<double> &B) {
+  const int n = A.r, k = A.c, nr = std::min(6, B.c);
+  int lhi = k - 1;
+  for (; lhi >= 0; --lhi) {
+    bool any = false;
+    for (int q = 0; q < nr; ++q) any = any || B.a[(size_t)q * k + lhi] != 0.0;
+    if (any) break;
+  }
+  matmul_block_f64<1>(c, A.a.data(), B.a.data(), n, k, 0, lhi);
+}
+inline void matmul_col0(std::complex<double> *c, const Mat<std::complex<double>> &A, const Mat<std::complex<double>> &B) {
+  const int n = A.r, k = A.c, nr = std::min(3, B.c);
+  const double *Bd = reinterpret_cast<const double *>(B.a.data());
+  int lhi = k - 1;
+  for (; lhi >= 0; --lhi) {
+    bool any = false;
+    for (int q = 0; q < nr; ++q) { const double *bp = Bd + 2 * ((size_t)q * k + lhi); any = any || bp[0] != 0.0 || bp[1] != 0.0; }
+    if (any) break;
+  }
+  matmul_block_c64<1>(reinterpret_cast<double *>(c), reinterpret_cast<const double *>(A.a.data()), Bd, n, k, 0, lhi);
+}
+#endif
 
 template <class S>
 inline real_t<S> opnorm1(const Mat<S> &A) {
@@ -501,9 +525,17 @@
 }
 
 template <class S>
-inline Mat<S> pade_evaluate(const Mat<S> &A, const double *C, int N) {
+struct ExpmWork {
+  Mat<S> A2, P, U, V, tmp, X, D, B;
+};
+template <class S>
+inline void pade_uv(const Mat<S> &A, const double *C, int N, ExpmWork<S> &w) {
   const int n = A.r;
-  Mat<S> A2, P(n, n), U(n, n), V(n, n), tmp;
+  Mat<S> &A2 = w.A2, &P = w.P, &U = w.U, &V = w.V, &tmp = w.tmp;
+  for (Mat<S> *M : {&P, &U, &V}) {
+    if (M->r != n || M->c != n) *M = Mat<S>(n, n);
+    else std::fill(M->a.begin(), M->a.end(), S(0));
+  }
   matmul(A2, A, A);
   typedef real_t<S> R;
   for (int i = 0; i < n; ++i) { P(i, i) = S(1); U(i, i) = S(R(C[1])); V(i, i) = S(R(C[0])); }
@@ -520,6 +552,13 @@
   }
   matmul(tmp, A, U);
   std::swap(U.a, tmp.a);
+}
+template <class S>
+inline Mat<S> pade_evaluate(const Mat<S> &A, const double *C, int N) {
+  const int n = A.r;
+  ExpmWork<S> w;
+  pade_uv(A, C, N, w);
+  const Mat<S> &U = w.U, &V = w.V;
   Mat<S> X(n, n), D(n, n);
   for (size_t i = 0; i < X.a.size(); ++i) { X.a[i] = V.a[i] + U.a[i]; D.a[i] = V.a[i] - U.a[i]; }
   lu_solve(D, X);
@@ -537,6 +576,36 @@
                                   40840800.0,          960960.0,            16380.0,
                                   182.0,               1.0};
 
+struct PadePlan { const double *C; int N; int squarings; };
+template <class S>
+inline PadePlan pade_plan(Mat<S> &A) {
+  typedef real_t<S> R;
+  const R nA = opnorm1(A);
+  if (nA <= R(2.1)) {
+    if (nA > R(0.95)) return PadePlan{PADE_C9, 10, 0};
+    if (nA > R(0.25)) return PadePlan{PADE_C7, 8, 0};
+    if (nA > R(0.015)) return PadePlan{PADE_C5, 6, 0};
+    return PadePlan{PADE_C3, 4, 0};
+  }
+  const R s = std::log2(nA / R(5.4));
+  int si = 0;
+  if (s > 0) {
+    si = (int)std::ceil(s);
+    const R sc = std::ldexp(R(1), si);
+    for (auto &v : A.a) v /= sc;
+  }
+  return PadePlan{PADE_C13, 14, si};
+}
+template <class S>
+inline Mat<S> expm_balanced(Mat<S> &A, const Balance<S> &bal) {
+  const PadePlan plan = pade_plan(A);
+  Mat<S> X = pade_evaluate(A, plan.C, plan.N);
+  Mat<S> tmp;
+  for (int t = 0; t < plan.squarings; ++t) { matmul(tmp, X, X); std::swap(X.a, tmp.a); }
+  unbalance(X, bal);
+  return X;
+}
+
 template <class S>
 inline void expm_higham2005base(Mat<S> &A) {
   typedef real_t<S> R;
@@ -546,29 +615,58 @@
     if (!std::isfinite(re_of(v)) || !std::isfinite(im_of(v)))
       throw std::invalid_argument("ArgumentError: matrix contains Infs or NaNs");
   Balance<S> bal = gebal(A);
-  const R nA = opnorm1(A);
-  Mat<S> X;
-  if (nA <= R(2.1)) {
-    if (nA > R(0.95)) X = pade_evaluate(A, PADE_C9, 10);
-    else if (nA > R(0.25)) X = pade_evaluate(A, PADE_C7, 8);
-    else if (nA > R(0.015)) X = pade_evaluate(A, PADE_C5, 6);
-    else X = pade_evaluate(A, PADE_C3, 4);
-  } else {
-    const R s = std::log2(nA / R(5.4));
-    int si = 0;
-    if (s > 0) {
-      si = (int)std::ceil(s);
-      const R sc = std::ldexp(R(1), si);
-      for (auto &v : A.a) v /= sc;
-    }
-    X = pade_evaluate(A, PADE_C13, 14);
-    if (s > 0) {
-      Mat<S> tmp;
-      for (int t = 0; t < si; ++t) { matmul(tmp, X, X); std::swap(X.a, tmp.a); }
-    }
-  }
-  unbalance(X, bal);
-  A = X;
+  A = expm_balanced(A, bal);
+}
+
+template <class S>
+inline void expm_higham2005base_col0(Mat<S> &A, S *out, ExpmWork<S> &w) {
+  const int n = A.r;
+  if (n == 0) return;
+  for (const auto &v : A.a)
+    if (!std::isfinite(re_of(v)) || !std::isfinite(im_of(v)))
+      throw std::invalid_argument("ArgumentError: matrix contains Infs or NaNs");
+  Balance<S> bal = gebal(A);
+#if defined(__AVX2__) && defined(__FMA__)
+  constexpr bool kernels = std::is_same<S, double>::value || std::is_same<S, std::complex<double>>::value;
+#else
+  constexpr bool kernels = false;
+#endif
+  if (!kernels || bal.ilo != 1 || bal.ihi != n) {
+    const Mat<S> X = expm_balanced(A, bal);
+    for (int i = 0; i < n; ++i) out[i] = X(i, 0);
+    return;
+  }
+#if defined(__AVX2__) && defined(__FMA__)
+  if constexpr (kernels) {
+    const PadePlan plan = pade_plan(A);
+    pade_uv(A, plan.C, plan.N, w);
+    const Mat<S> &U = w.U, &V = w.V;
+    Mat<S> &D = w.D;
+    if (D.r != n || D.c != n) D = Mat<S>(n, n);
+    for (size_t i = 0; i < D.a.size(); ++i) D.a[i] = V.a[i] - U.a[i];
+    if (plan.squarings == 0) {
+      const int nc = std::is_same<S, double>::value ? 1 : std::min(2, n);
+      Mat<S> &B = w.B;
+      if (B.r != n || B.c != nc) B = Mat<S>(n, nc);
+      for (size_t i = 0; i < B.a.size(); ++i) B.a[i] = V.a[i] + U.a[i];
+      lu_solve(D, B);
+      for (int i = 0; i < n; ++i) out[i] = B(i, 0);
+    } else {
+      Mat<S> &X = w.X, &tmp = w.tmp;
+      if (X.r != n || X.c != n) X = Mat<S>(n, n);
+      for (size_t i = 0; i < X.a.size(); ++i) X.a[i] = V.a[i] + U.a[i];
+      lu_solve(D, X);
+      for (int t = 0; t + 1 < plan.squarings; ++t) { matmul(tmp, X, X); std::swap(X.a, tmp.a); }
+      matmul_col0(out, X, X);
+    }
+    for (int j = 1; j <= n; ++j) {
+      const real_t<S> sj = bal.scale[j - 1];
+      out[j - 1] *= sj;
+      if (j == 1)
+        for (int i = 0; i < n; ++i) out[i] /= sj;
+    }
+  }
+#endif
 }
 
 template <bool ENDS_ONLY = false>
diff --git a/exponentialutilities.jl_amd/csrc/kernels.h b/exponentialutilities.jl_amd/csrc/kernels.h
--- a/exponentialutilities.jl_amd/csrc/kernels.h
+++ b/exponentialutilities.jl_amd/csrc/kernels.h
@@ -335,9 +335,11 @@
 template <class TC> struct CoefMat { TC c[COEF_MAT_MAX]; };
 template <class TV, class TC>
 void combine_v(hipStream_t s, int64_t n, const TV *V, int64_t ldv, int m, const CoefMat<TC> &cm, int ncols, double scale, TC *W, int64_t ldw);
+struct ZeroTwo { unsigned long long *a; size_t na; unsigned long long *b; size_t nb; };
 template <class TV, class TC>
 void combine1(hipStream_t s, int64_t n, const TV *V, int64_t ldv, int m, const CoefVec<TC> &cv, double scale, TC *W,
-              const int32_t *rowmap = nullptr);
+              const int32_t *rowmap = nullptr,
+              const ZeroTwo *zt = nullptr);
 template <class TC> struct LcTerms { int nterms; const TC *in[6]; TC coef[6]; double pscale; };
 template <class TV, class TC>
 void combine1_lc(hipStream_t s, int64_t n, const TV *V, int64_t ldv, int m, const CoefVec<TC> &cv, double scale, const LcTerms<TC> &lt, TC *W);
diff --git a/exponentialutilities.jl_amd/csrc/kernels.hip b/exponentialutilities.jl_amd/csrc/kernels.hip
--- a/exponentialutilities.jl_amd/csrc/kernels.hip
+++ b/exponentialutilities.jl_amd/csrc/kernels.hip
@@ -796,8 +796,12 @@
 template <class TV, class TC>
 __global__ __launch_bounds__(BLOCK) void k_combine1(int64_t n, const TV *__restrict__ V, int64_t ldv, int m,
                                                     CoefVec<TC> cv, double scale, TC *__restrict__ W, int64_t rpb,
-                                                    const int32_t *__restrict__ rowmap) {
+                                                    const int32_t *__restrict__ rowmap, ZeroTwo z) {
   constexpr int N = Pack<TV>::N;
+  for (size_t i = (size_t)blockIdx.x * BLOCK + threadIdx.x; i < z.na + z.nb; i += (size_t)gridDim.x * BLOCK) {
+    if (i < z.na) z.a[i] = 0ull;
+    else z.b[i - z.na] = 0ull;
+  }
   const bool al = ((ldv * sizeof(TV)) % 16 == 0) && is_al16(V);
   const int64_t r0 = (int64_t)blockIdx.x * rpb, r1 = (r0 + rpb < n) ? r0 + rpb : n;
   for (int64_t i = r0 + (int64_t)threadIdx.x * N; i < r1; i += (int64_t)BLOCK * N) {
@@ -825,10 +829,11 @@
   }
 }
 template <class TV, class TC>
-void combine1(hipStream_t s, int64_t n, const TV *V, int64_t ldv, int m, const CoefVec<TC> &cv, double scale, TC *W, const int32_t *rowmap) {
+void combine1(hipStream_t s, int64_t n, const TV *V, int64_t ldv, int m, const CoefVec<TC> &cv, double scale, TC *W, const int32_t *rowmap,
+              const ZeroTwo *zt) {
   const RowPlan p = plan_rows(n, 64 * Pack<TV>::N, resident_blocks((const void *)k_combine1<TV, TC>));
   hipLaunchKernelGGL((k_combine1<TV, TC>), dim3(p.nblocks), dim3(BLOCK), 0, s, n, V, ldv, m, cv, scale, W,
-                     p.rows_per_block, rowmap);
+                     p.rows_per_block, rowmap, zt ? *zt : ZeroTwo{nullptr, 0, nullptr, 0});
 }
 
 template <class TV, class TC>
@@ -964,9 +969,9 @@
                                         const LcTerms<float> &, float *);
 template void combine1_lc<cplx32, cplx32>(hipStream_t, int64_t, const cplx32 *, int64_t, int, const CoefVec<cplx32> &, double,
                                           const LcTerms<cplx32> &, cplx32 *);
-template void combine1<float, float>(hipStream_t, int64_t, const float *, int64_t, int, const CoefVec<float> &, double, float *, const int32_t *);
-template void combine1<float, cplx32>(hipStream_t, int64_t, const float *, int64_t, int, const CoefVec<cplx32> &, double, cplx32 *, const int32_t *);
-template void combine1<cplx32, cplx32>(hipStream_t, int64_t, const cplx32 *, int64_t, int, const CoefVec<cplx32> &, double, cplx32 *, const int32_t *);
+template void combine1<float, float>(hipStream_t, int64_t, const float *, int64_t, int, const CoefVec<float> &, double, float *, const int32_t *, const ZeroTwo *);
+template void combine1<float, cplx32>(hipStream_t, int64_t, const float *, int64_t, int, const CoefVec<cplx32> &, double, cplx32 *, const int32_t *, const ZeroTwo *);
+template void combine1<cplx32, cplx32>(hipStream_t, int64_t, const cplx32 *, int64_t, int, const CoefVec<cplx32> &, double, cplx32 *, const int32_t *, const ZeroTwo *);
 template void combine_v<float, float>(hipStream_t, int64_t, const float *, int64_t, int, const CoefMat<float> &, int, double, float *, int64_t);
 template void combine_v<float, cplx32>(hipStream_t, int64_t, const float *, int64_t, int, const CoefMat<cplx32> &, int, double, cplx32 *, int64_t);
 template void combine_v<cplx32, cplx32>(hipStream_t, int64_t, const cplx32 *, int64_t, int, const CoefMat<cplx32> &, int, double, cplx32 *, int64_t);
@@ -981,11 +986,11 @@
 template void combine1_lc<cplx, cplx>(hipStream_t, int64_t, const cplx *, int64_t, int, const CoefVec<cplx> &, double,
                                       const LcTerms<cplx> &, cplx *);
 template void combine1<double, double>(hipStream_t, int64_t, const double *, int64_t, int, const CoefVec<double> &,
-                                       double, double *, const int32_t *);
+                                       double, double *, const int32_t *, const ZeroTwo *);
 template void combine1<double, cplx>(hipStream_t, int64_t, const double *, int64_t, int, const CoefVec<cplx> &, double,
-                                     cplx *, const int32_t *);
+                                     cplx *, const int32_t *, const ZeroTwo *);
 template void combine1<cplx, cplx>(hipStream_t, int64_t, const cplx *, int64_t, int, const CoefVec<cplx> &, double,
-                                   cplx *, const int32_t *);
+                                   cplx *, const int32_t *, const ZeroTwo *);
 template void combine<double, double>(hipStream_t, int64_t, const double *, int64_t, int, const double *, int, int,
                                       double, double *, int64_t);
 template void combine<double, cplx>(hipStream_t, int64_t, const double *, int64_t, int, const cplx *, int, int, double,
diff --git a/include/expv_mi.h b/include/expv_mi.h
--- a/include/expv_mi.h
+++ b/include/expv_mi.h
@@ -40,6 +40,7 @@
 int expv_mi_ctx_set_option(expv_mi_ctx_t ctx, const char *name, int64_t value);
 int expv_mi_ctx_get_option(expv_mi_ctx_t ctx, const char *name, int64_t *value);
 int expv_mi_ctx_counters(expv_mi_ctx_t ctx, int64_t out[8]);
+int expv_mi_ctx_counters_more(expv_mi_ctx_t ctx, int64_t out[8]);
 int expv_mi_ctx_selftest(expv_mi_ctx_t ctx, int64_t out[8]);
 enum {
   EXPV_MI_PATH_MODULAR = 1, EXPV_MI_PATH_TWO_KERNEL = 2, EXPV_MI_PATH_PIPELINE = 4, EXPV_MI_PATH_WAVE = 8,
@@ -237,6 +238,7 @@
 int expv_mi_host_rcm(int64_t n, const int32_t *rowptr, const int32_t *colind, int dtype, int32_t *perm, int64_t out[4]);
 int expv_mi_host_wrapsum(const void *buf, uint64_t nbytes, uint64_t out[2]);
 int expv_mi_host_expm(int dtype, int n, void *A, int lda);
+int expv_mi_host_expm_col0(int dtype, int n, const void *A, int lda, void *col);
 int expv_mi_host_gebal(int dtype, int n, void *A, int lda, int64_t *ilo, int64_t *ihi, double *scale);
 int expv_mi_host_symtridiag_expcol(int n, const double *d, const double *e, double t_re, double t_im,
                                    double *out_c64);
```
